# AleoNet/snarkVM

Measured on AMD Instinct MI355X. Metric: BLS12-377 G1 MSM scalar-point pairs/sec (+ Fr NTT elements/sec in ntt_*), higher is better.
Workload: dtype u32 limbs (29-bit radix) modular integer arithmetic, Fq 377-bit / Fr 253-bit; 1 GPU; G1 Pippenger MSM 2^24 (BASELINE.json configs[1]), bases (i+1)G registered in HBM, uniform scalars in HBM; independent instance per GPU; scalars=uniform, lg_ntt=24, window_bits=auto, base_tables=12, table_bits=22, pipelined_batch=True

## Files before the change

include/snarkvm_hip.h:

```cpp
#ifndef SNARKVM_HIP_H
#define SNARKVM_HIP_H

#include <stddef.h>
#include <stdint.h>

#ifdef __cplusplus
extern "C" {
#endif

typedef struct {
    int32_t code;
    char *message;
} RustError;

enum NTTInputOutputOrder { NN = 0, NR = 1, RN = 2, RR = 3 };
enum NTTDirection { Forward = 0, Inverse = 1 };
enum NTTType { Standard = 0, Coset = 1 };


RustError snarkvm_ntt(void *inout, uint32_t lg_domain_size, enum NTTInputOutputOrder ntt_order,
                      enum NTTDirection ntt_direction, enum NTTType ntt_type);

RustError snarkvm_polymul(void *out, size_t pcount, const void *polynomials, const void *plens, size_t ecount,
                          const void *evaluations, const void *elens, uint32_t lg_domain_size);

RustError snarkvm_msm(void *out, const void *points_with_infinity, size_t npoints, const void *scalars,
                      size_t ffi_affine_sz);
RustError snarkvm_hip_set_base_cache(int tables);
RustError snarkvm_hip_set_base_cache_verified(int tables);
void snarkvm_hip_base_cache_stats(uint64_t *out, int reset);


int snarkvm_hip_device_count(void);
int snarkvm_hip_batch_lanes(size_t npoints);
RustError snarkvm_hip_set_devices(const int32_t *ids, size_t n);
RustError snarkvm_hip_set_device(int device);
int snarkvm_hip_num_devices(void);

RustError snarkvm_hip_malloc(void **d_ptr, size_t bytes, int device);
RustError snarkvm_hip_free(void *d_ptr);
RustError snarkvm_hip_memcpy_h2d(void *d_dst, const void *src, size_t bytes);
RustError snarkvm_hip_memcpy_d2h(void *dst, const void *d_src, size_t bytes);
RustError snarkvm_hip_memcpy_d2d(void *d_dst, const void *d_src, size_t bytes);
RustError snarkvm_hip_memset(void *d_dst, int value, size_t bytes);

RustError snarkvm_hip_ntt_device(void *d_inout, uint32_t lg_domain_size, int ntt_order, int ntt_direction,
                                 int ntt_type);
RustError snarkvm_hip_ntt_device_batch(void *const *d_inouts, size_t count, uint32_t lg_domain_size, int ntt_order,
                                       const int *ntt_directions, const int *ntt_types);

RustError snarkvm_hip_polymul_device(void *d_out, size_t pcount, const void *const *d_polys, const size_t *plens, size_t ecount,
                                     const void *const *d_evals, const size_t *elens, uint32_t lg_domain_size);

RustError snarkvm_hip_scope_begin(const void *d_any);
RustError snarkvm_hip_scope_end(void);
enum { SNARKVM_HIP_SCOPE_ASYNC_MSM = 1, SNARKVM_HIP_SCOPE_STABLE_INPUTS = 2, SNARKVM_HIP_SCOPE_MSM_IN_STREAM = 4 };
RustError snarkvm_hip_scope_begin_ex(const void *d_any, uint32_t flags);
RustError snarkvm_hip_scope_collect(const void *out);
RustError snarkvm_hip_scope_set_flags(uint32_t flags);
void *snarkvm_hip_scope_stream(void);

typedef struct snarkvm_hip_bases snarkvm_hip_bases_t;
RustError snarkvm_hip_register_bases(snarkvm_hip_bases_t **handle, const void *points, size_t npoints,
                                     size_t ffi_affine_sz, int on_device);
RustError snarkvm_hip_register_bases_tables(snarkvm_hip_bases_t **handle, const void *points, size_t npoints,
                                            size_t ffi_affine_sz, int on_device, int tables);
RustError snarkvm_hip_register_bases_windowed(snarkvm_hip_bases_t **handle, const void *points, size_t npoints,
                                              size_t ffi_affine_sz, int on_device, int tables, int window_bits);
void snarkvm_hip_free_bases(snarkvm_hip_bases_t *handle);

RustError snarkvm_hip_register_bases_serialized(snarkvm_hip_bases_t **handle, const void *bytes, size_t npoints,
                                                int compressed, int validate, int tables);
RustError snarkvm_hip_g1_deserialize(void *out_affine, const void *bytes, size_t n, int compressed, int validate);
RustError snarkvm_hip_g1_serialize(void *out_bytes, const void *affine, size_t n, size_t ffi_affine_sz, int compressed);

RustError snarkvm_hip_g2_deserialize(void *out_affine, const void *bytes, size_t n, int validate);
RustError snarkvm_hip_g2_serialize(void *out_bytes, const void *affine, size_t n, size_t ffi_affine_sz);
RustError snarkvm_hip_g2_deserialize_compressed(void *out_affine, const void *bytes, size_t n, int validate);
RustError snarkvm_hip_g2_serialize_compressed(void *out_bytes, const void *affine, size_t n, size_t ffi_affine_sz);

RustError snarkvm_hip_msm_registered(void *out, const snarkvm_hip_bases_t *handle, size_t offset, size_t npoints,
                                     const void *scalars, int scalars_on_device, int window_bits);

RustError snarkvm_hip_msm_registered_ex(void *out, const snarkvm_hip_bases_t *handle, size_t off0, size_t n0,
                                        size_t off1, size_t n1, const void *scalars, int scalars_on_device,
                                        int scalars_montgomery, int window_bits);

RustError snarkvm_hip_msm_registered_batch(void *outs, const snarkvm_hip_bases_t *handle, size_t count,
                                           const size_t *offsets, const size_t *npoints, const void *const *scalars,
                                           int scalars_on_device, int scalars_montgomery, int window_bits);

RustError snarkvm_hip_msm_registered_batch_ex(void *outs, const snarkvm_hip_bases_t *handle, size_t count, const size_t *off0,
                                              const size_t *n0, const size_t *off1, const size_t *n1,
                                              const void *const *scalars, int scalars_on_device, int scalars_montgomery,
                                              int window_bits);

RustError snarkvm_hip_g1_sum(void *out, const void *in_projective, size_t n);

RustError snarkvm_hip_g1_to_affine(void *out_affine, const void *in_projective, size_t n);

RustError snarkvm_hip_msm_g2(void *out, const void *points_with_infinity, size_t npoints, const void *scalars,
                             size_t ffi_affine_sz);

typedef struct snarkvm_hip_bases_g2 snarkvm_hip_bases_g2_t;
RustError snarkvm_hip_register_bases_g2(snarkvm_hip_bases_g2_t **handle, const void *points, size_t npoints,
                                        size_t ffi_affine_sz, int tables, int window_bits);
void snarkvm_hip_free_bases_g2(snarkvm_hip_bases_g2_t *handle);
RustError snarkvm_hip_msm_g2_registered(void *out, const snarkvm_hip_bases_g2_t *handle, size_t offset, size_t npoints,
                                        const void *scalars, int scalars_on_device, int window_bits);
RustError snarkvm_hip_msm_g2_registered_batch(void *outs, const snarkvm_hip_bases_g2_t *handle, size_t count,
                                              const size_t *offsets, const size_t *npoints, const void *const *scalars,
                                              int scalars_on_device, int window_bits);

RustError snarkvm_hip_g1_fixed_base_msm(void *out_projective, const void *g_affine, const void *scalars, size_t n);
RustError snarkvm_hip_g1_group_ntt(void *inout_projective, uint32_t lg_domain_size, int inverse);

RustError snarkvm_hip_fr_mul_device(void *d_out, const void *d_a, const void *d_b, size_t n);
RustError snarkvm_hip_fr_convert_device(void *d_out, const void *d_in, size_t n, int to_bigint);

RustError snarkvm_hip_fr_vec_op(int op, void *out, const void *a, const void *b, const void *c, const void *scalar,
                                size_t n, int on_device);
RustError snarkvm_hip_fr_divide_by_linear(void *quotient, void *remainder, const void *poly, size_t n,
                                          const void *point, int on_device);
RustError snarkvm_hip_fr_batch_inversion_and_mul(void *inout, size_t n, const void *coeff, int on_device);
RustError snarkvm_hip_fr_distribute_powers(void *inout, size_t n, const void *g, const void *c, int on_device);
RustError snarkvm_hip_fr_lagrange_coefficients(void *out, uint32_t lg_domain_size, const void *tau, int on_device);
RustError snarkvm_hip_fr_divide_by_vanishing(void *quotient, void *remainder, const void *poly, size_t len,
                                             size_t domain_size, int on_device);
RustError snarkvm_hip_fr_mul_by_vanishing(void *out, const void *poly, size_t len, size_t domain_size, int on_device);

RustError snarkvm_hip_fr_lincomb(void *out, size_t n_out, size_t count, const void *const *polys, const size_t *lens, const void *coeffs,
                                 int on_device);

RustError snarkvm_hip_fr_vec_op_strided(int op, void *out, const void *a, const void *b, const void *c, const void *scalar,
                                        size_t n, size_t count, size_t stride);
RustError snarkvm_hip_fr_divide_by_linear_strided(void *quotients, void *remainders, const void *polys, size_t n,
                                                  const void *point, size_t count, size_t stride);
RustError snarkvm_hip_fr_divide_by_vanishing_strided(void *quotients, void *remainders, const void *polys, size_t len,
                                                     size_t domain_size, size_t count, size_t stride);

RustError snarkvm_hip_g1_generate_bases_device(void *d_out, uint64_t start, size_t npoints);

void snarkvm_hip_set_profiling(int enabled);
int snarkvm_hip_get_phase_count(void);
const char *snarkvm_hip_get_phase_name(int i);
double snarkvm_hip_get_phase_ms(int i);

void snarkvm_hip_coalescer_stats(uint64_t *out, int reset);

void snarkvm_hip_alloc_stats(uint64_t *out, int reset);

RustError snarkvm_hip_synchronize(void);


int snarkvm_hip_selftest_field(int field, int op, const void *a, const void *b, void *out, size_t n);
int snarkvm_hip_selftest_g1_msm_naive(const void *points_with_infinity, size_t npoints, size_t ffi_affine_sz,
                                      const void *scalars, void *out);
int snarkvm_hip_selftest_msm_plan(size_t n, int window_bits, int tables, int table_bits, uint32_t *out);
int snarkvm_hip_selftest_g1_finish(const void *planes_projective, const int32_t *pos, size_t n, void *out);
int snarkvm_hip_selftest_fq_lazy(uint64_t seed, int iters);
int snarkvm_hip_selftest_g1_lazy_tail(uint64_t seed, int iters);
int snarkvm_hip_selftest_fq2_pair(const void *points, size_t npoints, uint64_t seed, int iters);
int snarkvm_hip_selftest_g2_hex(const void *points, size_t npoints, uint64_t seed, int iters);
RustError snarkvm_hip_devtest_g2_tail_repeat(const void *points, size_t npoints, int m, int hb, int threads, int plane_threads,
                                             int hex, int quads, int iters, uint32_t *report);
int snarkvm_hip_selftest_ntt_plan(uint32_t lg, int32_t *out);
int snarkvm_hip_selftest_ntt_twiddle(int kind, uint32_t lg, int pass, int inverse, const uint64_t *x, size_t n, void *out);
int snarkvm_hip_selftest_ntt_index(uint32_t lg, const int32_t *plan, int npass);
int snarkvm_hip_selftest_ntt_host(void *inout, uint32_t lg, const int32_t *plan, int npass, int dir, int type);
int snarkvm_hip_selftest_fr_lincomb(void *out, size_t n_out, size_t count, const void *const *polys, const size_t *lens, const void *coeffs);
RustError snarkvm_hip_devtest_field(int field, int op, const void *a, const void *b, void *out, size_t n);

#ifdef __cplusplus
}
#endif
#endif
```

rust/snarkvm-algorithms-hip/src/sys.rs:

```rust
#![allow(non_camel_case_types, non_snake_case, clippy::too_many_arguments, clippy::missing_safety_doc)]
use super::{Error, NTTDirection, NTTInputOutputOrder, NTTType};
use core::ffi::{c_char, c_void};

#[repr(C)]
pub struct snarkvm_hip_bases_t {
    _private: [u8; 0],
}
#[repr(C)]
pub struct snarkvm_hip_bases_g2_t {
    _private: [u8; 0],
}

pub const SNARKVM_HIP_SCOPE_ASYNC_MSM: u32 = 1;
pub const SNARKVM_HIP_SCOPE_STABLE_INPUTS: u32 = 2;
pub const SNARKVM_HIP_SCOPE_MSM_IN_STREAM: u32 = 4;

extern "C" {
    pub fn snarkvm_ntt(inout: *mut c_void, lg_domain_size: u32, ntt_order: NTTInputOutputOrder, ntt_direction: NTTDirection, ntt_type: NTTType) -> Error;
    pub fn snarkvm_polymul(out: *mut c_void, pcount: usize, polynomials: *const c_void, plens: *const c_void, ecount: usize, evaluations: *const c_void, elens: *const c_void, lg_domain_size: u32) -> Error;
    pub fn snarkvm_msm(out: *mut c_void, points_with_infinity: *const c_void, npoints: usize, scalars: *const c_void, ffi_affine_sz: usize) -> Error;
    pub fn snarkvm_hip_set_base_cache(tables: i32) -> Error;
    pub fn snarkvm_hip_set_base_cache_verified(tables: i32) -> Error;
    pub fn snarkvm_hip_base_cache_stats(out: *mut u64, reset: i32);
    pub fn snarkvm_hip_device_count() -> i32;
    pub fn snarkvm_hip_batch_lanes(npoints: usize) -> i32;
    pub fn snarkvm_hip_set_devices(ids: *const i32, n: usize) -> Error;
    pub fn snarkvm_hip_set_device(device: i32) -> Error;
    pub fn snarkvm_hip_num_devices() -> i32;
    pub fn snarkvm_hip_malloc(d_ptr: *mut *mut c_void, bytes: usize, device: i32) -> Error;
    pub fn snarkvm_hip_free(d_ptr: *mut c_void) -> Error;
    pub fn snarkvm_hip_memcpy_h2d(d_dst: *mut c_void, src: *const c_void, bytes: usize) -> Error;
    pub fn snarkvm_hip_memcpy_d2h(dst: *mut c_void, d_src: *const c_void, bytes: usize) -> Error;
    pub fn snarkvm_hip_memcpy_d2d(d_dst: *mut c_void, d_src: *const c_void, bytes: usize) -> Error;
    pub fn snarkvm_hip_memset(d_dst: *mut c_void, value: i32, bytes: usize) -> Error;
    pub fn snarkvm_hip_ntt_device(d_inout: *mut c_void, lg_domain_size: u32, ntt_order: i32, ntt_direction: i32, ntt_type: i32) -> Error;
    pub fn snarkvm_hip_ntt_device_batch(d_inouts: *const *mut c_void, count: usize, lg_domain_size: u32, ntt_order: i32, ntt_directions: *const i32, ntt_types: *const i32) -> Error;
    pub fn snarkvm_hip_polymul_device(d_out: *mut c_void, pcount: usize, d_polys: *const *const c_void, plens: *const usize, ecount: usize, d_evals: *const *const c_void, elens: *const usize, lg_domain_size: u32) -> Error;
    pub fn snarkvm_hip_scope_begin(d_any: *const c_void) -> Error;
    pub fn snarkvm_hip_scope_end() -> Error;
    pub fn snarkvm_hip_scope_begin_ex(d_any: *const c_void, flags: u32) -> Error;
    pub fn snarkvm_hip_scope_collect(out: *const c_void) -> Error;
    pub fn snarkvm_hip_scope_set_flags(flags: u32) -> Error;
    pub fn snarkvm_hip_scope_stream() -> *mut c_void;
    pub fn snarkvm_hip_register_bases(handle: *mut *mut snarkvm_hip_bases_t, points: *const c_void, npoints: usize, ffi_affine_sz: usize, on_device: i32) -> Error;
    pub fn snarkvm_hip_register_bases_tables(handle: *mut *mut snarkvm_hip_bases_t, points: *const c_void, npoints: usize, ffi_affine_sz: usize, on_device: i32, tables: i32) -> Error;
    pub fn snarkvm_hip_register_bases_windowed(handle: *mut *mut snarkvm_hip_bases_t, points: *const c_void, npoints: usize, ffi_affine_sz: usize, on_device: i32, tables: i32, window_bits: i32) -> Error;
    pub fn snarkvm_hip_free_bases(handle: *mut snarkvm_hip_bases_t);
    pub fn snarkvm_hip_register_bases_serialized(handle: *mut *mut snarkvm_hip_bases_t, bytes: *const c_void, npoints: usize, compressed: i32, validate: i32, tables: i32) -> Error;
    pub fn snarkvm_hip_g1_deserialize(out_affine: *mut c_void, bytes: *const c_void, n: usize, compressed: i32, validate: i32) -> Error;
    pub fn snarkvm_hip_g1_serialize(out_bytes: *mut c_void, affine: *const c_void, n: usize, ffi_affine_sz: usize, compressed: i32) -> Error;
    pub fn snarkvm_hip_g2_deserialize(out_affine: *mut c_void, bytes: *const c_void, n: usize, validate: i32) -> Error;
    pub fn snarkvm_hip_g2_serialize(out_bytes: *mut c_void, affine: *const c_void, n: usize, ffi_affine_sz: usize) -> Error;
    pub fn snarkvm_hip_g2_deserialize_compressed(out_affine: *mut c_void, bytes: *const c_void, n: usize, validate: i32) -> Error;
    pub fn snarkvm_hip_g2_serialize_compressed(out_bytes: *mut c_void, affine: *const c_void, n: usize, ffi_affine_sz: usize) -> Error;
    pub fn snarkvm_hip_msm_registered(out: *mut c_void, handle: *const snarkvm_hip_bases_t, offset: usize, npoints: usize, scalars: *const c_void, scalars_on_device: i32, window_bits: i32) -> Error;
    pub fn snarkvm_hip_msm_registered_ex(out: *mut c_void, handle: *const snarkvm_hip_bases_t, off0: usize, n0: usize, off1: usize, n1: usize, scalars: *const c_void, scalars_on_device: i32, scalars_montgomery: i32, window_bits: i32) -> Error;
    pub fn snarkvm_hip_msm_registered_batch(outs: *mut c_void, handle: *const snarkvm_hip_bases_t, count: usize, offsets: *const usize, npoints: *const usize, scalars: *const *const c_void, scalars_on_device: i32, scalars_montgomery: i32, window_bits: i32) -> Error;
    pub fn snarkvm_hip_msm_registered_batch_ex(outs: *mut c_void, handle: *const snarkvm_hip_bases_t, count: usize, off0: *const usize, n0: *const usize, off1: *const usize, n1: *const usize, scalars: *const *const c_void, scalars_on_device: i32, scalars_montgomery: i32, window_bits: i32) -> Error;
    pub fn snarkvm_hip_g1_sum(out: *mut c_void, in_projective: *const c_void, n: usize) -> Error;
    pub fn snarkvm_hip_g1_to_affine(out_affine: *mut c_void, in_projective: *const c_void, n: usize) -> Error;
    pub fn snarkvm_hip_msm_g2(out: *mut c_void, points_with_infinity: *const c_void, npoints: usize, scalars: *const c_void, ffi_affine_sz: usize) -> Error;
    pub fn snarkvm_hip_register_bases_g2(handle: *mut *mut snarkvm_hip_bases_g2_t, points: *const c_void, npoints: usize, ffi_affine_sz: usize, tables: i32, window_bits: i32) -> Error;
    pub fn snarkvm_hip_free_bases_g2(handle: *mut snarkvm_hip_bases_g2_t);
    pub fn snarkvm_hip_msm_g2_registered(out: *mut c_void, handle: *const snarkvm_hip_bases_g2_t, offset: usize, npoints: usize, scalars: *const c_void, scalars_on_device: i32, window_bits: i32) -> Error;
    pub fn snarkvm_hip_msm_g2_registered_batch(outs: *mut c_void, handle: *const snarkvm_hip_bases_g2_t, count: usize, offsets: *const usize, npoints: *const usize, scalars: *const *const c_void, scalars_on_device: i32, window_bits: i32) -> Error;
    pub fn snarkvm_hip_g1_fixed_base_msm(out_projective: *mut c_void, g_affine: *const c_void, scalars: *const c_void, n: usize) -> Error;
    pub fn snarkvm_hip_g1_group_ntt(inout_projective: *mut c_void, lg_domain_size: u32, inverse: i32) -> Error;
    pub fn snarkvm_hip_fr_mul_device(d_out: *mut c_void, d_a: *const c_void, d_b: *const c_void, n: usize) -> Error;
    pub fn snarkvm_hip_fr_convert_device(d_out: *mut c_void, d_in: *const c_void, n: usize, to_bigint: i32) -> Error;
    pub fn snarkvm_hip_fr_vec_op(op: i32, out: *mut c_void, a: *const c_void, b: *const c_void, c: *const c_void, scalar: *const c_void, n: usize, on_device: i32) -> Error;
    pub fn snarkvm_hip_fr_divide_by_linear(quotient: *mut c_void, remainder: *mut c_void, poly: *const c_void, n: usize, point: *const c_void, on_device: i32) -> Error;
    pub fn snarkvm_hip_fr_batch_inversion_and_mul(inout: *mut c_void, n: usize, coeff: *const c_void, on_device: i32) -> Error;
    pub fn snarkvm_hip_fr_distribute_powers(inout: *mut c_void, n: usize, g: *const c_void, c: *const c_void, on_device: i32) -> Error;
    pub fn snarkvm_hip_fr_lagrange_coefficients(out: *mut c_void, lg_domain_size: u32, tau: *const c_void, on_device: i32) -> Error;
    pub fn snarkvm_hip_fr_divide_by_vanishing(quotient: *mut c_void, remainder: *mut c_void, poly: *const c_void, len: usize, domain_size: usize, on_device: i32) -> Error;
    pub fn snarkvm_hip_fr_mul_by_vanishing(out: *mut c_void, poly: *const c_void, len: usize, domain_size: usize, on_device: i32) -> Error;
    pub fn snarkvm_hip_fr_lincomb(out: *mut c_void, n_out: usize, count: usize, polys: *const *const c_void, lens: *const usize, coeffs: *const c_void, on_device: i32) -> Error;
    pub fn snarkvm_hip_fr_vec_op_strided(op: i32, out: *mut c_void, a: *const c_void, b: *const c_void, c: *const c_void, scalar: *const c_void, n: usize, count: usize, stride: usize) -> Error;
    pub fn snarkvm_hip_fr_divide_by_linear_strided(quotients: *mut c_void, remainders: *mut c_void, polys: *const c_void, n: usize, point: *const c_void, count: usize, stride: usize) -> Error;
    pub fn snarkvm_hip_fr_divide_by_vanishing_strided(quotients: *mut c_void, remainders: *mut c_void, polys: *const c_void, len: usize, domain_size: usize, count: usize, stride: usize) -> Error;
    pub fn snarkvm_hip_g1_generate_bases_device(d_out: *mut c_void, start: u64, npoints: usize) -> Error;
    pub fn snarkvm_hip_set_profiling(enabled: i32);
    pub fn snarkvm_hip_get_phase_count() -> i32;
    pub fn snarkvm_hip_get_phase_name(i: i32) -> *const c_char;
    pub fn snarkvm_hip_get_phase_ms(i: i32) -> f64;
    pub fn snarkvm_hip_coalescer_stats(out: *mut u64, reset: i32);
    pub fn snarkvm_hip_alloc_stats(out: *mut u64, reset: i32);
    pub fn snarkvm_hip_synchronize() -> Error;
    pub fn snarkvm_hip_selftest_field(field: i32, op: i32, a: *const c_void, b: *const c_void, out: *mut c_void, n: usize) -> i32;
    pub fn snarkvm_hip_selftest_g1_msm_naive(points_with_infinity: *const c_void, npoints: usize, ffi_affine_sz: usize, scalars: *const c_void, out: *mut c_void) -> i32;
    pub fn snarkvm_hip_selftest_msm_plan(n: usize, window_bits: i32, tables: i32, table_bits: i32, out: *mut u32) -> i32;
    pub fn snarkvm_hip_selftest_g1_finish(planes_projective: *const c_void, pos: *const i32, n: usize, out: *mut c_void) -> i32;
    pub fn snarkvm_hip_selftest_fq_lazy(seed: u64, iters: i32) -> i32;
    pub fn snarkvm_hip_selftest_g1_lazy_tail(seed: u64, iters: i32) -> i32;
    pub fn snarkvm_hip_selftest_fq2_pair(points: *const c_void, npoints: usize, seed: u64, iters: i32) -> i32;
    pub fn snarkvm_hip_selftest_g2_hex(points: *const c_void, npoints: usize, seed: u64, iters: i32) -> i32;
    pub fn snarkvm_hip_devtest_g2_tail_repeat(points: *const c_void, npoints: usize, m: i32, hb: i32, threads: i32, plane_threads: i32, hex: i32, quads: i32, iters: i32, report: *mut u32) -> Error;
    pub fn snarkvm_hip_selftest_ntt_plan(lg: u32, out: *mut i32) -> i32;
    pub fn snarkvm_hip_selftest_ntt_twiddle(kind: i32, lg: u32, pass: i32, inverse: i32, x: *const u64, n: usize, out: *mut c_void) -> i32;
    pub fn snarkvm_hip_selftest_ntt_index(lg: u32, plan: *const i32, npass: i32) -> i32;
    pub fn snarkvm_hip_selftest_ntt_host(inout: *mut c_void, lg: u32, plan: *const i32, npass: i32, dir: i32, type_: i32) -> i32;
    pub fn snarkvm_hip_selftest_fr_lincomb(out: *mut c_void, n_out: usize, count: usize, polys: *const *const c_void, lens: *const usize, coeffs: *const c_void) -> i32;
    pub fn snarkvm_hip_devtest_field(field: i32, op: i32, a: *const c_void, b: *const c_void, out: *mut c_void, n: usize) -> Error;
}
```

snarkvm_amd/_lib.py:

```python
import ctypes
import os

_HERE = os.path.dirname(os.path.abspath(__file__))
LIB_PATH = os.environ.get("SNARKVM_HIP_LIB") or os.path.join(_HERE, "lib", "libsnarkvm_hip.so")

SYMBOLS = [
    "snarkvm_ntt", "snarkvm_polymul", "snarkvm_msm", "snarkvm_hip_set_base_cache", "snarkvm_hip_set_base_cache_verified", "snarkvm_hip_base_cache_stats",
    "snarkvm_hip_device_count", "snarkvm_hip_batch_lanes", "snarkvm_hip_set_device", "snarkvm_hip_set_devices", "snarkvm_hip_num_devices",
    "snarkvm_hip_malloc", "snarkvm_hip_free", "snarkvm_hip_memcpy_h2d", "snarkvm_hip_memcpy_d2h", "snarkvm_hip_memcpy_d2d", "snarkvm_hip_memset", "snarkvm_hip_ntt_device", "snarkvm_hip_ntt_device_batch", "snarkvm_hip_polymul_device",
    "snarkvm_hip_scope_begin", "snarkvm_hip_scope_end", "snarkvm_hip_scope_begin_ex", "snarkvm_hip_scope_collect", "snarkvm_hip_scope_set_flags", "snarkvm_hip_scope_stream", "snarkvm_hip_alloc_stats",
    "snarkvm_hip_register_bases", "snarkvm_hip_register_bases_tables", "snarkvm_hip_register_bases_windowed", "snarkvm_hip_free_bases", "snarkvm_hip_msm_registered", "snarkvm_hip_msm_g2",
    "snarkvm_hip_msm_registered_ex", "snarkvm_hip_msm_registered_batch", "snarkvm_hip_msm_registered_batch_ex", "snarkvm_hip_g1_to_affine",
    "snarkvm_hip_fr_mul_device", "snarkvm_hip_fr_convert_device", "snarkvm_hip_g1_generate_bases_device",
    "snarkvm_hip_fr_vec_op", "snarkvm_hip_fr_divide_by_linear", "snarkvm_hip_fr_batch_inversion_and_mul",
    "snarkvm_hip_fr_distribute_powers", "snarkvm_hip_fr_lagrange_coefficients", "snarkvm_hip_fr_divide_by_vanishing",
    "snarkvm_hip_fr_mul_by_vanishing", "snarkvm_hip_fr_lincomb",
    "snarkvm_hip_fr_vec_op_strided", "snarkvm_hip_fr_divide_by_linear_strided", "snarkvm_hip_fr_divide_by_vanishing_strided",
    "snarkvm_hip_register_bases_serialized", "snarkvm_hip_g1_deserialize", "snarkvm_hip_g1_serialize", "snarkvm_hip_g1_sum", "snarkvm_hip_g2_deserialize", "snarkvm_hip_g2_serialize", "snarkvm_hip_g2_deserialize_compressed", "snarkvm_hip_g2_serialize_compressed",
    "snarkvm_hip_register_bases_g2", "snarkvm_hip_free_bases_g2", "snarkvm_hip_msm_g2_registered", "snarkvm_hip_msm_g2_registered_batch",
    "snarkvm_hip_g1_fixed_base_msm", "snarkvm_hip_g1_group_ntt",
    "snarkvm_hip_set_profiling", "snarkvm_hip_get_phase_count", "snarkvm_hip_get_phase_name",
    "snarkvm_hip_get_phase_ms", "snarkvm_hip_synchronize", "snarkvm_hip_coalescer_stats",
    "snarkvm_hip_selftest_field", "snarkvm_hip_selftest_g1_msm_naive", "snarkvm_hip_selftest_msm_plan", "snarkvm_hip_selftest_g1_finish", "snarkvm_hip_selftest_fq_lazy", "snarkvm_hip_selftest_g1_lazy_tail", "snarkvm_hip_selftest_ntt_plan", "snarkvm_hip_selftest_ntt_twiddle", "snarkvm_hip_selftest_ntt_index", "snarkvm_hip_selftest_ntt_host", "snarkvm_hip_selftest_fq2_pair", "snarkvm_hip_selftest_g2_hex", "snarkvm_hip_selftest_fr_lincomb", "snarkvm_hip_devtest_field", "snarkvm_hip_devtest_g2_tail_repeat",
]


class RustError(ctypes.Structure):
    _fields_ = [("code", ctypes.c_int32), ("message", ctypes.c_void_p)]


class HipError(RuntimeError):
    def __init__(self, code, message):
        super().__init__(f"snarkvm_hip error {code}: {message}")
        self.code = code
        self.message = message


_lib = None
_libc = None


def lib():
    global _lib, _libc
    if _lib is None:
        if not os.path.exists(LIB_PATH):
            raise ImportError(
                f"{LIB_PATH} is missing - build it with `python -m snarkvm_amd.build` (hipcc, gfx950). "
                "snarkvm_amd has no CPU fallback.")
        if not os.environ.get("SNARKVM_HIP_NO_TORCH"):
            try:
                import torch
            except ImportError:
                pass
        L = ctypes.CDLL(LIB_PATH)
        err_fns = ["snarkvm_ntt", "snarkvm_polymul", "snarkvm_msm", "snarkvm_hip_set_base_cache", "snarkvm_hip_set_base_cache_verified", "snarkvm_hip_set_device", "snarkvm_hip_set_devices",
                   "snarkvm_hip_malloc", "snarkvm_hip_free", "snarkvm_hip_memcpy_h2d", "snarkvm_hip_memcpy_d2h", "snarkvm_hip_memcpy_d2d", "snarkvm_hip_memset", "snarkvm_hip_ntt_device", "snarkvm_hip_ntt_device_batch", "snarkvm_hip_polymul_device",
                   "snarkvm_hip_scope_begin", "snarkvm_hip_scope_end", "snarkvm_hip_scope_begin_ex", "snarkvm_hip_scope_collect", "snarkvm_hip_scope_set_flags",
                   "snarkvm_hip_register_bases", "snarkvm_hip_register_bases_tables", "snarkvm_hip_register_bases_windowed", "snarkvm_hip_msm_registered", "snarkvm_hip_msm_g2", "snarkvm_hip_msm_registered_ex", "snarkvm_hip_msm_registered_batch", "snarkvm_hip_msm_registered_batch_ex", "snarkvm_hip_g1_to_affine", "snarkvm_hip_fr_mul_device",
                   "snarkvm_hip_fr_convert_device", "snarkvm_hip_g1_generate_bases_device", "snarkvm_hip_synchronize",
                   "snarkvm_hip_fr_vec_op", "snarkvm_hip_fr_divide_by_linear", "snarkvm_hip_fr_batch_inversion_and_mul", "snarkvm_hip_fr_distribute_powers", "snarkvm_hip_fr_lagrange_coefficients", "snarkvm_hip_fr_divide_by_vanishing", "snarkvm_hip_fr_mul_by_vanishing", "snarkvm_hip_fr_lincomb",
                   "snarkvm_hip_fr_vec_op_strided", "snarkvm_hip_fr_divide_by_linear_strided", "snarkvm_hip_fr_divide_by_vanishing_strided",
                   "snarkvm_hip_register_bases_serialized", "snarkvm_hip_g1_deserialize", "snarkvm_hip_g1_serialize", "snarkvm_hip_g1_sum", "snarkvm_hip_g2_deserialize", "snarkvm_hip_g2_serialize", "snarkvm_hip_g2_deserialize_compressed", "snarkvm_hip_g2_serialize_compressed",
                   "snarkvm_hip_register_bases_g2", "snarkvm_hip_msm_g2_registered", "snarkvm_hip_msm_g2_registered_batch",
                   "snarkvm_hip_g1_fixed_base_msm", "snarkvm_hip_g1_group_ntt",
                   "snarkvm_hip_devtest_field", "snarkvm_hip_devtest_g2_tail_repeat"]
        for name in err_fns:
            getattr(L, name).restype = RustError
        L.snarkvm_hip_device_count.restype = ctypes.c_int
        L.snarkvm_hip_batch_lanes.restype = ctypes.c_int
        L.snarkvm_hip_num_devices.restype = ctypes.c_int
        L.snarkvm_hip_selftest_g1_finish.restype = ctypes.c_int
        L.snarkvm_hip_selftest_fq_lazy.restype = ctypes.c_int
        L.snarkvm_hip_selftest_g1_lazy_tail.restype = ctypes.c_int
        for name in ("snarkvm_hip_selftest_ntt_plan", "snarkvm_hip_selftest_ntt_twiddle", "snarkvm_hip_selftest_ntt_index", "snarkvm_hip_selftest_ntt_host"):
            getattr(L, name).restype = ctypes.c_int
        L.snarkvm_hip_selftest_fq2_pair.restype = ctypes.c_int
        L.snarkvm_hip_selftest_g2_hex.restype = ctypes.c_int
        L.snarkvm_hip_selftest_fr_lincomb.restype = ctypes.c_int
        L.snarkvm_hip_get_phase_count.restype = ctypes.c_int
        L.snarkvm_hip_get_phase_name.restype = ctypes.c_char_p
        L.snarkvm_hip_get_phase_ms.restype = ctypes.c_double
        L.snarkvm_hip_selftest_field.restype = ctypes.c_int
        L.snarkvm_hip_selftest_g1_msm_naive.restype = ctypes.c_int
        L.snarkvm_hip_selftest_msm_plan.restype = ctypes.c_int
        L.snarkvm_hip_free_bases.restype = None
        L.snarkvm_hip_free_bases_g2.restype = None
        L.snarkvm_hip_set_profiling.restype = None
        L.snarkvm_hip_coalescer_stats.restype = None
        L.snarkvm_hip_base_cache_stats.restype = None
        L.snarkvm_hip_alloc_stats.restype = None
        L.snarkvm_hip_scope_stream.restype = ctypes.c_void_p
        L.snarkvm_hip_scope_begin_ex.argtypes = [ctypes.c_void_p, ctypes.c_uint32]
        L.snarkvm_hip_scope_set_flags.argtypes = [ctypes.c_uint32]
        L.snarkvm_hip_alloc_stats.argtypes = [ctypes.c_void_p, ctypes.c_int]
        L.snarkvm_hip_coalescer_stats.argtypes = [ctypes.c_void_p, ctypes.c_int]
        L.snarkvm_hip_base_cache_stats.argtypes = [ctypes.c_void_p, ctypes.c_int]
        L.snarkvm_hip_malloc.argtypes = [ctypes.POINTER(ctypes.c_void_p), ctypes.c_size_t, ctypes.c_int]
        L.snarkvm_hip_free.argtypes = [ctypes.c_void_p]
        L.snarkvm_hip_memcpy_h2d.argtypes = [ctypes.c_void_p, ctypes.c_void_p, ctypes.c_size_t]
        L.snarkvm_hip_memcpy_d2h.argtypes = [ctypes.c_void_p, ctypes.c_void_p, ctypes.c_size_t]
        L.snarkvm_hip_memcpy_d2d.argtypes = [ctypes.c_void_p, ctypes.c_void_p, ctypes.c_size_t]
        L.snarkvm_hip_memset.argtypes = [ctypes.c_void_p, ctypes.c_int, ctypes.c_size_t]
        L.snarkvm_hip_polymul_device.argtypes = [ctypes.c_void_p, ctypes.c_size_t, ctypes.POINTER(ctypes.c_void_p), ctypes.POINTER(ctypes.c_size_t),
                                                 ctypes.c_size_t, ctypes.POINTER(ctypes.c_void_p), ctypes.POINTER(ctypes.c_size_t), ctypes.c_uint32]
        L.snarkvm_hip_fr_lincomb.argtypes = [ctypes.c_void_p, ctypes.c_size_t, ctypes.c_size_t, ctypes.POINTER(ctypes.c_void_p), ctypes.POINTER(ctypes.c_size_t),
                                             ctypes.c_void_p, ctypes.c_int]
        L.snarkvm_hip_selftest_fr_lincomb.argtypes = L.snarkvm_hip_fr_lincomb.argtypes[:-1]
        _libc = ctypes.CDLL(None)
        _libc.free.argtypes = [ctypes.c_void_p]
        _lib = L
    return _lib


def check(err):
    if err.code != 0:
        msg = ctypes.string_at(err.message).decode(errors="replace") if err.message else ""
        if err.message:
            _libc.free(err.message)
        raise HipError(err.code, msg)


def device_count():
    return lib().snarkvm_hip_device_count()
```

snarkvm_amd/csrc/api.hip:

```cpp
#define SV_TU_G1
#include "runtime.hip.h"
#include "ffl.hip.h"

runtime_t g_rt;
thread_local thread_scope_t g_tl_scope;
thread_scope_t::~thread_scope_t() {
    if (!lane) return;
    pending.clear();
    (void)hipStreamSynchronize(lane->stream);
    for (int i = 0; i < naux; i++) {
        (void)hipStreamSynchronize(aux[i]->stream);
        aux[i]->dev->give(aux[i], true);
    }
    lane->in_scope = false;
    lane->deferred.clear();
    lane->deferred_bytes = 0;
    if (!lane->tw_leases.empty()) ntt_tw_release(lane->dev, lane->tw_leases);
    lane->dev->give(lane, true);
    lane = nullptr;
}
std::atomic<uint64_t> g_co_stats[4];
static std::atomic<uint64_t> g_alloc_stats[5];
void sv_alloc_note(int slot, size_t bytes, double ms) {
    g_alloc_stats[slot].fetch_add(1, std::memory_order_relaxed);
// ... 153 lines not shown
    c.sync_or_defer();
    API_END
}

static constexpr uint32_t SCOPE_FLAGS_ALL = SNARKVM_HIP_SCOPE_ASYNC_MSM | SNARKVM_HIP_SCOPE_STABLE_INPUTS | SNARKVM_HIP_SCOPE_MSM_IN_STREAM;
RustError snarkvm_hip_scope_begin_ex(const void* d_any, uint32_t flags) {
    API_TRY
    thread_scope_t& sc = tl_scope();
    if (sc.lane) throw hip_failure{hipErrorInvalidValue, "scope_begin: the calling thread already has an open scope", __LINE__};
    if (flags & ~SCOPE_FLAGS_ALL) throw hip_failure{hipErrorInvalidValue, "scope_begin: unknown flag", __LINE__};
    g_rt.configure();
    const int nd = (int)g_rt.devs.size();
    int dev = device_for(d_any, d_any ? 1 : 0);
    if (dev < 0) dev = (int)(g_rt.rr.fetch_add(1) % (uint32_t)nd);
    device_t* d = g_rt.devs[dev].get();
    int prev = -1;
    if (hipGetDevice(&prev) != hipSuccess) prev = 0;
    lane_t* l = d->take_for_scope(true);
    try {
        HIP_TRY(hipSetDevice(d->physical));
        d->init();
        tu_kernel_attributes(d->logical);
    } catch (...) {
        d->give(l, true);
        (void)hipSetDevice(prev);
        throw;
    }
    l->begin_call();
    l->in_scope = true;
    l->pin_used = 0;
    l->scope_events_used = 0;
    sc = thread_scope_t();
    sc.lane = l;
    sc.prev_device = prev;
    sc.flags = flags;
    API_CATCH
}
RustError snarkvm_hip_scope_begin(const void* d_any) { return snarkvm_hip_scope_begin_ex(d_any, 0); }
void* snarkvm_hip_scope_stream(void) {
    lane_t* l = tl_scope().lane;
    return l ? (void*)l->stream : nullptr;
}
RustError snarkvm_hip_scope_set_flags(uint32_t flags) {
    API_TRY
    thread_scope_t& sc = tl_scope();
    if (!sc.lane) throw hip_failure{hipErrorInvalidValue, "scope_set_flags: the calling thread has no open scope", __LINE__};
    if (flags & ~SCOPE_FLAGS_ALL) throw hip_failure{hipErrorInvalidValue, "scope_set_flags: unknown flag", __LINE__};
    sc.flags = flags;
    API_CATCH
}
RustError snarkvm_hip_scope_collect(const void* out) {
    API_TRY
    scope_collect(out);
    API_CATCH
}
RustError snarkvm_hip_scope_end(void) {
    thread_scope_t& sc = tl_scope();
    lane_t* l = sc.lane;
    if (!l) return ok();
    RustError r = ok();
    try {
        scope_flush();
    } catch (const hip_failure& f) {
        r = from_failure(f);
    } catch (const std::exception& e) {
        r = fail(1, std::string("snarkvm_hip: scope_end: ") + e.what());
    } catch (...) {
        r = fail(1, "snarkvm_hip: scope_end failed");
    }
    l->in_scope = false;
    l->deferred.clear();
    l->deferred_bytes = 0;
    for (int i = 0; i < sc.naux; i++) {
        (void)hipStreamSynchronize(sc.aux[i]->stream);
        sc.aux[i]->dev->give(sc.aux[i], true);
    }
    const int prev = sc.prev_device;
    sc = thread_scope_t();
    l->dev->give(l, true);
    if (prev >= 0) (void)hipSetDevice(prev);
    return r;
}

static void precompute_tables(lane_t& c, snarkvm_hip_bases* h, g1_aff_mem_t* d) { precompute_tables_run<fq_t>(c, d, h->n, h->tables, h->table_bits); }
static void register_bases_impl(snarkvm_hip_bases_t** handle, const void* points, size_t npoints, size_t ffi_affine_sz, int on_device, int tables,
                                int table_bits) {
    if (!handle) throw hip_failure{hipErrorInvalidValue, "register_bases: null handle", __LINE__};
    if (npoints && !points) throw hip_failure{hipErrorInvalidValue, "register_bases: null points", __LINE__};
    if (ffi_affine_sz < 104 || (ffi_affine_sz & 7)) throw hip_failure{hipErrorInvalidValue, "register_bases: bad stride", __LINE__};
    check_tables(tables, table_bits, "register_bases");
    scope_flush();
    const int nd = g_rt.ndev();
    std::unique_ptr<snarkvm_hip_bases> h(new snarkvm_hip_bases());
    h->n = npoints;
    h->tables = tables;
    h->table_bits = table_bits ? table_bits : 256 / tables;
    h->d.assign(nd, nullptr);
    const size_t bytes = (size_t)tables * npoints * sizeof(g1_aff_mem_t);
    try {
        if (npoints) {
            const int owner = on_device ? device_for(points, 1) : -1;
            auto build = [&](int dev) {
                lane_guard lg(dev);
                lane_t& c = lg.c();
                HIP_TRY(hipMalloc((void**)&h->d[dev], bytes));
                const uint8_t* src = (const uint8_t*)points;
                if (!on_device) {
                    c.bases_tmp.ensure(npoints * ffi_affine_sz);
                    HIP_TRY(hipMemcpyAsync(c.bases_tmp.p, points, npoints * ffi_affine_sz, hipMemcpyHostToDevice, c.stream));
                    src = c.bases_tmp.as<uint8_t>();
                }
                convert_bases<fq_t>(c, src, ffi_affine_sz, npoints, h->d[dev]);
                precompute_tables(c, h.get(), h->d[dev]);
                bases_to_lazy_form(c, h->d[dev], (size_t)tables * npoints);
                HIP_TRY(hipStreamSynchronize(c.stream));
            };
            std::vector<int> all;
            for (int d = 0; d < nd; d++) all.push_back(d);
            if (!on_device) {
                for_each_device(all, build);
            } else {
                build(owner);
                for (int d = 0; d < nd; d++) {
                    if (d == owner) continue;
                    lane_guard lg(d);
                    HIP_TRY(hipMalloc((void**)&h->d[d], bytes));
                    HIP_TRY(hipMemcpyPeerAsync(h->d[d], g_rt.devs[d]->physical, h->d[owner], g_rt.devs[owner]->physical, bytes, lg.c().stream));
                    HIP_TRY(hipStreamSynchronize(lg.c().stream));
                }
            }
        }
    } catch (...) {
        h->free_all();
        throw;
    }
    *handle = h.release();
}
RustError snarkvm_hip_register_bases(snarkvm_hip_bases_t** handle, const void* points, size_t npoints, size_t ffi_affine_sz, int on_device) {
    API_TRY
    register_bases_impl(handle, points, npoints, ffi_affine_sz, on_device, 1, 0);
    API_CATCH
}
RustError snarkvm_hip_register_bases_tables(snarkvm_hip_bases_t** handle, const void* points, size_t npoints, size_t ffi_affine_sz, int on_device,
                                            int tables) {
    API_TRY
    register_bases_impl(handle, points, npoints, ffi_affine_sz, on_device, tables, 0);
    API_CATCH
}
RustError snarkvm_hip_register_bases_windowed(snarkvm_hip_bases_t** handle, const void* points, size_t npoints, size_t ffi_affine_sz, int on_device,
                                              int tables, int window_bits) {
    API_TRY
    if (window_bits <= 0) throw hip_failure{hipErrorInvalidValue, "register_bases_windowed: window_bits must be positive", __LINE__};
    register_bases_impl(handle, points, npoints, ffi_affine_sz, on_device, tables, window_bits);
    API_CATCH
}
void snarkvm_hip_free_bases(snarkvm_hip_bases_t* h) {
    if (!h) return;
    h->free_all();
    delete h;
}
}
snarkvm_hip_bases* sv_new_bases_handle(size_t npoints, int tables, int table_bits) {
    snarkvm_hip_bases* h = new snarkvm_hip_bases();
    h->n = npoints;
    h->tables = tables;
    h->table_bits = table_bits;
    h->d.assign(g_rt.ndev(), nullptr);
    return h;
}
void sv_precompute_tables(lane_t& c, snarkvm_hip_bases* h, g1_aff_mem_t* d) { precompute_tables(c, h, d); }
extern "C" {

static void check_window_bits(int window_bits, const char* who) {
    if (window_bits && (window_bits < 2 || window_bits > MSM_C_MAX)) throw std::runtime_error(std::string(who) + ": window_bits must be 0 or 2..23");
}
static void msm_registered_host_scalars(void* out, const snarkvm_hip_bases* h, size_t off0, size_t n0, size_t off1, size_t n1, const void* scalars,
                                        int scalars_montgomery, int window_bits) {
    const size_t n = n0 + n1;
    scope_flush();
    const int nd = g_rt.ndev();
    static const int trace = getenv("SNARKVM_HIP_TRACE") ? atoi(getenv("SNARKVM_HIP_TRACE")) : 0;
    const double t_begin = host_now_ms();
    size_t parts = n / MSM_SPLIT_MIN;
    if (parts > (size_t)nd) parts = (size_t)nd;
    if (parts < 1) parts = 1;
    const size_t chunk = msm_scalar_chunk_pairs();
    if (n >= 2 * chunk && (n + chunk - 1) / chunk > parts) parts = (n + chunk - 1) / chunk;
    std::vector<size_t> bound;
    const int geo = tuning().scalar_geo;
    if (nd == 1 && geo > 1 && tuning().taper != 0 && n >= ((size_t)1 << 22)) {
        parts = n >= ((size_t)1 << 23) ? 3 : 2;
        size_t wsum = 0, w = 1;
        for (size_t i = 0; i < parts; i++, w *= (size_t)geo) wsum += w;
        size_t acc_w = 0;
        w = 1;
        bound.push_back(0);
        for (size_t i = 0; i < parts; i++, w *= (size_t)geo) {
            acc_w += w;
            bound.push_back(i + 1 == parts ? n : (size_t)((unsigned __int128)n * acc_w / wsum));
        }
    } else {
        for (size_t i = 0; i <= parts; i++) bound.push_back(n * i / parts);
    }
    const int ndu = (int)(parts < (size_t)nd ? parts : (size_t)nd);
    std::unique_ptr<msm_accum_t<fq_t>> acc(new msm_accum_t<fq_t>());
    std::mutex acc_mu;
    std::vector<int> devs;
    if (ndu == 1) {
        devs.push_back(-1);
    } else {
        for (int d = 0; d < ndu; d++) devs.push_back(d);
    }
    const size_t slot = msm_plane_bytes<fq_t>();
    for_each_device(devs, [&](int dev) {
        std::vector<size_t> mine;
        for (size_t i = (dev < 0 ? 0 : (size_t)dev); i < parts; i += (size_t)ndu) mine.push_back(i);
        lane_guard lg;
        lg.acquire(dev, mine.size() > 2 ? 3 : (int)mine.size());
        const size_t L = lg.lanes.size();
        size_t max_cnt = 0;
        for (size_t j = 0; j < mine.size(); j++) {
            const size_t cnt = bound[mine[j] + 1] - bound[mine[j]];
            max_cnt = cnt > max_cnt ? cnt : max_cnt;
        }
        const bool use_sink = tuning().taper != 0 && mine.size() >= 2;
        std::vector<msm_pending_t> pend(use_sink ? 1 : mine.size());
        int chunk_c = window_bits;
        msm_bucket_sink_t sink;
        std::vector<hipEvent_t> merged;
        for (size_t l = 0; l < L; l++) {
            lane_t& c = *lg.lanes[l];
            c.begin_call();
            c.scalars_tmp.ensure(max_cnt * 32 + 32);
            c.pin.ensure(slot * (use_sink ? 1 : (mine.size() + L - 1) / L));
        }
        if (use_sink) {
            lane_t& c0 = *lg.lanes[0];
            const msm_plan_t pl = msm_make_plan(max_cnt, window_bits, h->tables, h->table_bits);
// ... 615 lines not shown
        }
    }
    const g1_jac_t j = total.to_jacobian();
    uint32_t* o = (uint32_t*)out;
    j.x.to_mem_mont().pack(o);
    j.y.to_mem_mont().pack(o + 12);
    j.z.to_mem_mont().pack(o + 24);
    return 0;
}
int snarkvm_hip_selftest_fq_lazy(uint64_t seed, int iters) {
    uint32_t xw[12], yw[12];
    memcpy(xw, G1_GEN_X, 48);
    memcpy(yw, G1_GEN_Y, 48);
    const g1_aff_t g{fq_t::unpack(xw).from_mem_mont(), fq_t::unpack(yw).from_mem_mont()};
    std::vector<g1_aff_t> pool;
    g1_xyzz_t run = g1_xyzz_t::inf();
    for (int k = 0; k < 64; k++) {
        run.add_affine(g);
        const fq_t izzz = run.zzz.inverse();
        const fq_t izz = izzz.sqr() * run.zz.sqr();
        pool.push_back({run.x * izz, run.y * izzz});
    }
    const fq_t c406 = fq_t::from_table(FqLConv::C406), c348 = fq_t::from_table(FqLConv::C348);
    auto next = [&]() {
        seed += 0x9E3779B97F4A7C15ull;
        uint64_t z = seed;
        z = (z ^ (z >> 30)) * 0xBF58476D1CE4E5B9ull;
        z = (z ^ (z >> 27)) * 0x94D049BB133111EBull;
        return z ^ (z >> 31);
    };
    g1_xyzz_t exact = g1_xyzz_t::inf();
    xyzz_lazy_t lazy = xyzz_lazy_t::infinity();
    int prev = -1;
    bool prev_neg = false;
    for (int it = 0; it < iters; it++) {
        const uint64_t r = next();
        int k = (int)(r % 64);
        bool neg = ((r >> 8) & 1) != 0;
        const int mode = (int)((r >> 16) % 16);
        if (mode == 0 && prev >= 0) k = prev, neg = prev_neg;
        if (mode == 1 && prev >= 0) k = prev, neg = !prev_neg;
        if (mode == 2) {
            exact = g1_xyzz_t::inf();
            lazy = xyzz_lazy_t::infinity();
        }
        prev = k;
        prev_neg = neg;
        const g1_aff_t p = pool[k];
        exact.add_affine(p, neg);
        const fql_t px = fql_t::from_limbs(p.x * c406), py = fql_t::from_limbs(p.y * c406);
        if (!lazy.madd(px, py, neg)) {
            g1_xyzz_t e = lazy.to_exact();
            fq_t ex, ey;
            for (int i = 0; i < 13; i++) ex.v[i] = (uint32_t)px.v[i], ey.v[i] = (uint32_t)py.v[i];
            e.add_affine({ex * c348, ey * c348}, neg);
            lazy = xyzz_lazy_t::from_exact(e);
        }
        const g1_xyzz_t got = lazy.to_exact();
        if (got.is_inf() != exact.is_inf()) return it + 1;
        if (!exact.is_inf() && (got.x != exact.x || got.y != exact.y || got.zz != exact.zz || got.zzz != exact.zzz)) return it + 1;
    }
    for (int t = 0; t < 200; t++) {
        fq_t a, b;
        for (int i = 0; i < 13; i++) a.v[i] = (uint32_t)(next() & LIMB_MASK), b.v[i] = (uint32_t)(next() & LIMB_MASK);
        a.v[12] &= 0x00ffffffu;
        b.v[12] &= 0x00ffffffu;
        if (t & 1) for (int i = 0; i < 12; i++) a.v[i] = LIMB_MASK;
        if (t & 2) for (int i = 0; i < 12; i++) b.v[i] = (i & 1) ? LIMB_MASK : 0;
        const fql_t la = fql_t::from_exact(a), lb = fql_t::from_exact(b);
        if (fql_t::mul(la, lb).to_exact() != a * b) return -(4 * t + 1);
        if (fql_t::sqr(la - lb).to_exact() != (a - b).sqr()) return -(4 * t + 2);
        if (fql_t::diff_of_products(la - lb, lb - la, fql_t::from_exact(a * b).normalized(), la).to_exact() != fq_t::diff_of_products(a - b, b - a, a * b, a))
            return -(4 * t + 3);
        if (((la + lb) - (lb + lb)).normalized().to_exact() != (a - b)) return -(4 * t + 4);
        alignas(16) uint32_t raw[12];
        const fql_t wide = (la - lb - lb - lb).normalized();
        wide.store_raw(raw);
        const fql_t back = fql_t::load_raw(raw);
        for (int i = 0; i < 13; i++)
            if (back.v[i] != wide.v[i]) return -(100000 + t);
    }
    return 0;
}
int snarkvm_hip_selftest_g1_lazy_tail(uint64_t seed, int iters) {
    uint32_t xw[12], yw[12];
    memcpy(xw, G1_GEN_X, 48);
    memcpy(yw, G1_GEN_Y, 48);
    const g1_aff_t g{fq_t::unpack(xw).from_mem_mont(), fq_t::unpack(yw).from_mem_mont()};
    std::vector<g1_xyzz_t> pool;
    g1_xyzz_t run = g1_xyzz_t::inf();
    for (int k = 0; k < 48; k++) {
        run.add_affine(g);
        pool.push_back(run);
    }
    auto next = [&]() {
        seed += 0x9E3779B97F4A7C15ull;
        uint64_t z = seed;
        z = (z ^ (z >> 30)) * 0xBF58476D1CE4E5B9ull;
        z = (z ^ (z >> 27)) * 0x94D049BB133111EBull;
        return z ^ (z >> 31);
    };
    auto to_lazy = [](const g1_xyzz_t& p) {
        xyzz_t<fqz_t> r = xyzz_t<fqz_t>::inf();
        if (!p.is_inf()) r = {{fql_t::from_exact(p.x)}, {fql_t::from_exact(p.y)}, {fql_t::from_exact(p.zz)}, {fql_t::from_exact(p.zzz)}};
        return r;
    };
    g1_xyzz_t exact = g1_xyzz_t::inf();
    xyzz_t<fqz_t> lazy = xyzz_t<fqz_t>::inf();
    g1_xyzz_t prev = g1_xyzz_t::inf();
    for (int it = 0; it < iters; it++) {
        const uint64_t r = next();
        g1_xyzz_t p = pool[r % 48];
        fq_t l = fq_t::zero();
        for (int i = 0; i < 12; i++) l.v[i] = (uint32_t)(next() & LIMB_MASK);
        l.v[0] |= 1;
        const fq_t l2 = l.sqr(), l3 = l2 * l;
        p = {p.x * l2, p.y * l3, p.zz * l2, p.zzz * l3};
        if ((r >> 8) & 1) p.y = p.y.neg();
        const int mode = (int)((r >> 16) % 16);
        if (mode == 0) p = prev;
        if (mode == 1) p = {prev.x, prev.y.neg(), prev.zz, prev.zzz};
        if (mode == 2) {
            exact = g1_xyzz_t::inf();
            lazy = xyzz_t<fqz_t>::inf();
        }
        if (mode == 3) p = exact;
        if (mode == 4) {
            exact = exact.dbl();
            lazy = lazy.dbl();
        } else {
            prev = p;
            exact.add(p);
            lazy.add(to_lazy(p));
        }
        if (lazy.is_inf() != exact.is_inf()) return it + 1;
        if (!exact.is_inf() && (lazy.x.to_exact() != exact.x || lazy.y.to_exact() != exact.y || lazy.zz.to_exact() != exact.zz || lazy.zzz.to_exact() != exact.zzz))
            return it + 1;
        xyzz_mem_t<fqz_t> m;
        store_xyzz<fqz_t>(&m, lazy);
        lazy = load_xyzz<fqz_t>(&m);
    }
    fqz_t zq;
    for (int i = 0; i < 13; i++) zq.a.v[i] = FqL::MOD[i];
    if (!zq.is_zero() || !zq.neg().is_zero() || !(zq + zq).is_zero() || (zq + fqz_t::one()).is_zero()) return -1;
    return 0;
}
int snarkvm_hip_selftest_g1_finish(const void* planes_jacobian, const int32_t* pos, size_t n, void* out) {
    try {
        std::unique_ptr<msm_accum_t<fq_t>> acc(new msm_accum_t<fq_t>());
        const uint32_t* src = (const uint32_t*)planes_jacobian;
        for (size_t i = 0; i < n; i++) {
            const g1_jac_t j = {fq_t::from_raw_words(src + 36 * i), fq_t::from_raw_words(src + 36 * i + 12), fq_t::from_raw_words(src + 36 * i + 24)};
            acc->add(pos[i], g1_xyzz_t::from_jacobian(j));
        }
        acc->finish(out);
        return 0;
    } catch (...) {
        return 1;
    }
}

}
```

snarkvm_amd/csrc/api_serde.hip:

```cpp
#include "runtime.hip.h"

snarkvm_hip_bases* sv_new_bases_handle(size_t npoints, int tables, int table_bits);
void sv_precompute_tables(lane_t& c, snarkvm_hip_bases* h, g1_aff_mem_t* d);

static uint32_t g1_deserialize_run(lane_t& c, const void* bytes, size_t n, int compressed, int validate, g1_aff_mem_t* d_native, uint8_t* d_rust) {
    const size_t psz = compressed ? 48 : 96;
    c.bases_tmp.ensure(n * psz);
    c.serde_status.ensure(4);
    HIP_TRY(hipMemcpyAsync(c.bases_tmp.p, bytes, n * psz, hipMemcpyHostToDevice, c.stream));
    HIP_TRY(hipMemsetAsync(c.serde_status.p, 0, 4, c.stream));
    hipLaunchKernelGGL(g1_deserialize_kernel, dim3((unsigned)((n + 63) / 64)), dim3(64), 0, c.stream, c.bases_tmp.as<uint8_t>(), n, compressed, validate,
                       d_native, d_rust, c.serde_status.as<uint32_t>());
    HIP_TRY(hipGetLastError());
    uint32_t st = 0;
    HIP_TRY(hipMemcpyAsync(&st, c.serde_status.p, 4, hipMemcpyDeviceToHost, c.stream));
    HIP_TRY(hipStreamSynchronize(c.stream));
    return st;
}

extern "C" {

RustError snarkvm_hip_register_bases_serialized(snarkvm_hip_bases_t** handle, const void* bytes, size_t npoints, int compressed, int validate,
                                                int tables) {
    API_TRY
    if (!handle || (npoints && !bytes)) throw hip_failure{hipErrorInvalidValue, "register_bases_serialized: null argument", __LINE__};
    check_tables(tables, 0, "register_bases_serialized");
    std::unique_ptr<snarkvm_hip_bases> h(sv_new_bases_handle(npoints, tables, 256 / tables));
    if (npoints) {
        try {
            std::vector<int> all;
            for (int d = 0; d < g_rt.ndev(); d++) all.push_back(d);
            for_each_device(all, [&](int dev) {
                lane_guard lg(dev);
                lane_t& c = lg.c();
                HIP_TRY(hipMalloc((void**)&h->d[dev], (size_t)tables * npoints * sizeof(g1_aff_mem_t)));
                serde_throw_on_status(g1_deserialize_run(c, bytes, npoints, compressed, validate, h->d[dev], nullptr), "register_bases_serialized");
                sv_precompute_tables(c, h.get(), h->d[dev]);
                bases_to_lazy_form(c, h->d[dev], (size_t)tables * npoints);
                HIP_TRY(hipStreamSynchronize(c.stream));
            });
        } catch (...) {
            h->free_all();
            throw;
        }
    }
    *handle = h.release();
    API_CATCH
}
RustError snarkvm_hip_g1_deserialize(void* out_affine, const void* bytes, size_t n, int compressed, int validate) {
    API_BEGIN
    if (n) {
        if (!out_affine || !bytes) throw hip_failure{hipErrorInvalidValue, "g1_deserialize: null argument", __LINE__};
        c.poly[0].ensure(n * 104);
        const uint32_t st = g1_deserialize_run(c, bytes, n, compressed, validate, nullptr, c.poly[0].as<uint8_t>());
        serde_throw_on_status(st, "g1_deserialize");
        HIP_TRY(hipMemcpyAsync(out_affine, c.poly[0].p, n * 104, hipMemcpyDeviceToHost, c.stream));
        HIP_TRY(hipStreamSynchronize(c.stream));
    }
    API_END
}
RustError snarkvm_hip_g1_serialize(void* out_bytes, const void* affine, size_t n, size_t ffi_affine_sz, int compressed) {
    API_BEGIN
    if (n) {
        if (!out_bytes || !affine) throw hip_failure{hipErrorInvalidValue, "g1_serialize: null argument", __LINE__};
        if (ffi_affine_sz < 104 || (ffi_affine_sz & 7)) throw hip_failure{hipErrorInvalidValue, "g1_serialize: bad stride", __LINE__};
        const size_t psz = compressed ? 48 : 96;
        c.bases_tmp.ensure(n * ffi_affine_sz);
        c.poly[0].ensure(n * psz);
        HIP_TRY(hipMemcpyAsync(c.bases_tmp.p, affine, n * ffi_affine_sz, hipMemcpyHostToDevice, c.stream));
        hipLaunchKernelGGL(g1_serialize_kernel, dim3((unsigned)((n + 63) / 64)), dim3(64), 0, c.stream, c.bases_tmp.as<uint8_t>(), ffi_affine_sz, n,
                           compressed, c.poly[0].as<uint8_t>());
        HIP_TRY(hipGetLastError());
        HIP_TRY(hipMemcpyAsync(out_bytes, c.poly[0].p, n * psz, hipMemcpyDeviceToHost, c.stream));
        HIP_TRY(hipStreamSynchronize(c.stream));
    }
    API_END
}

}
```

snarkvm_amd/csrc/msm_sort.hip.h:

```cpp
#pragma once
#include "ffl.hip.h"
#include "ffl2.hip.h"
#include "ffl2p.hip.h"
#include "msm.hip.h"

namespace sv {

static constexpr int SORT_TILE = 8192;
static constexpr int SORT_THREADS = 256;

struct msm_inst_t {
    const uint4* scalars;
    uint32_t n;
    uint32_t n0;
    uint32_t off0, off1;
    uint32_t pstart;
    uint32_t ptiles;
};
struct msm_radix_params_t {
    size_t n;
    int c, W, J;
    int HB, LB;
    uint32_t nb;
    uint32_t tiles_per_row;
    uint32_t TPW;
    const msm_inst_t* inst = nullptr;
    uint32_t ninst = 0;
    uint32_t vstride = 0, vn0 = 0, vr0 = 0, vr1 = 0;
    uint32_t xcd = 0;
};
__device__ __forceinline__ uint32_t xcd_tile(uint32_t b, uint32_t T) {
    const uint32_t q = T >> 3, r = T & 7u, x = b & 7u;
    return (x < r ? x * (q + 1) : r * (q + 1) + (x - r) * q) + (b >> 3);
}
struct l1_tile_t {
    uint32_t w, tw, TPW, j;
    size_t cbase;
    size_t row;
    size_t lo, hi;
    uint32_t inst_idx;
};
__device__ __forceinline__ l1_tile_t l1_decode_tile(const msm_radix_params_t& p, uint32_t g) {
    l1_tile_t t;
    const uint32_t B1 = 1u << p.HB;
    if (!p.inst) {
        t.w = g / p.TPW;
        t.tw = g - t.w * p.TPW;
        t.TPW = p.TPW;
        t.j = t.tw / p.tiles_per_row;
        const uint32_t tt = t.tw - t.j * p.tiles_per_row;
        t.cbase = (size_t)t.w * B1 * p.TPW;
        t.row = (size_t)(t.j * p.W + t.w) * p.n;
        t.lo = (size_t)tt * SORT_TILE;
        t.hi = (t.lo + SORT_TILE < p.n) ? t.lo + SORT_TILE : p.n;
        t.inst_idx = 0;
        return t;
    }
    const uint32_t J = (uint32_t)p.J;
    uint32_t lo = 0, hi = p.ninst;
    while (hi - lo > 1) {
        const uint32_t mid = (lo + hi) >> 1;
        if (J * (p.inst[mid].pstart / SORT_TILE) <= g) lo = mid; else hi = mid;
    }
    const msm_inst_t in = p.inst[lo];
    const uint32_t tw0 = J * (in.pstart / SORT_TILE);
    t.w = lo;
    t.inst_idx = lo;
    t.tw = g - tw0;
    t.TPW = J * in.ptiles;
    t.j = t.tw / in.ptiles;
    const uint32_t tt = t.tw - t.j * in.ptiles;
    t.cbase = (size_t)B1 * tw0;
    t.row = (size_t)t.j * p.n;
    t.lo = (size_t)in.pstart + (size_t)tt * SORT_TILE;
    t.hi = t.lo + SORT_TILE;
    return t;
}

__device__ __forceinline__ bool digit_bucket(uint32_t u, int half, uint32_t& b, uint32_t& neg) {
    const int dv = (int)u - half;
    if (dv == 0) return false;
    neg = dv < 0 ? 0x80000000u : 0u;
    b = (uint32_t)((dv < 0 ? -dv : dv) - 1);
    return true;
}

// ... 631 lines not shown
            raw = raw_next;
            if (pos + 1 < hi) {
                e_next = sorted[pos + 1];
                raw_next = *slot_of(e_next);
            }
        } else {
            raw = *slot_of(e);
            if (pos + 1 < hi) e_next = sorted[pos + 1];
        }
        acc.add_affine(load_aff<F>(&raw), (e >> 31) != 0);
    }
    store_xyzz<F>(&partial[start_k + part_off], acc);
}

static __global__ void __launch_bounds__(256) g1_partials_to_exact_kernel(const g1_lazy_partial_t* __restrict__ raw, g1_xyzz_mem_t* __restrict__ partial,
                                                                   const uint32_t* __restrict__ start, uint32_t nbt) {
    const uint32_t i = blockIdx.x * blockDim.x + threadIdx.x;
    if (i >= start[nbt]) return;
    g1_store_xyzz(&partial[i], xyzz_lazy_t::exact_from_raw(&raw[i]));
}
static __device__ __noinline__ void lazy_exceptional_add(xyzz_lazy_t* acc, const fql_t* px, const fql_t* py, bool neg) {
    g1_xyzz_t ex = acc->to_exact();
    const fq_t c348 = fq_t::from_table(FqLConv::C348);
    fq_t bx, by;
#pragma unroll
    for (int i = 0; i < 13; i++) bx.v[i] = (uint32_t)px->v[i], by.v[i] = (uint32_t)py->v[i];
    ex.add_affine({bx * c348, by * c348}, neg);
    *acc = xyzz_lazy_t::from_exact(ex);
}
template <bool PREFETCH>
__global__ void __launch_bounds__(256, 1) msm_accumulate_lazy_kernel(const g1_aff_mem_t* __restrict__ bases, const uint32_t* __restrict__ sorted,
                                                              const uint32_t* __restrict__ boff, const uint32_t* __restrict__ start,
                                                              g1_lazy_partial_t* __restrict__ partial, uint32_t nbt, uint32_t S, uint32_t debug_idx_mask) {
    const uint32_t t = blockIdx.x * blockDim.x + threadIdx.x;
    const uint32_t total = boff[nbt];
    const uint64_t lo64 = (uint64_t)t * S;
    if (lo64 >= total) return;
    const uint32_t lo = (uint32_t)lo64;
    const uint32_t hi = (total - lo < S) ? total : lo + S;
    uint32_t k = find_bucket(boff, nbt, lo);
    uint32_t kend = boff[k + 1];
    uint32_t kend2 = boff[k + 2 <= nbt ? k + 2 : nbt];
    uint32_t start_k = start[k];
    uint32_t part_off = t - boff[k] / S;
    xyzz_lazy_t acc = xyzz_lazy_t::infinity();
    auto slot_of = [&](uint32_t e) -> const g1_lazy_slot_t* { return (const g1_lazy_slot_t*)&bases[(e & 0x7fffffffu) & debug_idx_mask]; };
    uint32_t e_cur = sorted[lo];
    uint32_t e_n1 = lo + 1 < hi ? sorted[lo + 1] : 0u;
    g1_lazy_slot_t raw_next = *slot_of(e_cur);
    for (uint32_t pos = lo;; pos++) {
        const bool end = pos >= hi;
        if (end || pos >= kend) {
            acc.store_raw(&partial[start_k + part_off]);
            if (end) break;
            part_off = 0;
            acc.inf = true;
            k++;
            kend = kend2;
            while (pos >= kend) {
                k++;
                kend = boff[k + 1];
            }
            kend2 = boff[k + 2 <= nbt ? k + 2 : nbt];
            start_k = start[k];
        }
        const uint32_t e = e_cur;
        const g1_lazy_slot_t raw = raw_next;
        if (pos + 1 < hi) raw_next = *slot_of(e_n1);
        e_cur = e_n1;
        if (pos + 2 < hi) e_n1 = sorted[pos + 2];
        if (raw.w[26]) continue;
        const bool neg = (e >> 31) != 0;
        fql_t px, py;
        raw.coords(px, py);
        if (!acc.madd(px, py, neg)) {
            xyzz_lazy_t tmp = acc;
            const fql_t tx = px, ty = py;
            lazy_exceptional_add(&tmp, &tx, &ty, neg);
            acc = tmp;
        }
    }
}

static __global__ void __launch_bounds__(256) g2_pair_partials_to_exact_kernel(const g2_pair_partial_t* __restrict__ raw, xyzz_mem_t<fq2_t>* __restrict__ partial,
                                                                        const uint32_t* __restrict__ start, uint32_t nbt) {
    const uint32_t g = blockIdx.x * blockDim.x + threadIdx.x;
    const uint32_t i = g >> 3, k = g & 7;
    if (i >= start[nbt]) return;
    const uint4* q = (const uint4*)&raw[i].w[16 * k];
    uint32_t t[16];
#pragma unroll
    for (int j = 0; j < 4; j++) {
        const uint4 u = q[j];
        t[4 * j] = u.x, t[4 * j + 1] = u.y, t[4 * j + 2] = u.z, t[4 * j + 3] = u.w;
    }
    fql_t c;
#pragma unroll
    for (int j = 0; j < 13; j++) c.v[j] = (int32_t)t[j];
    c.to_exact().store(&((fq_mem_t*)&partial[i])[k]);
}
template <bool PREFETCH>
__global__ void __launch_bounds__(256, 2) msm_accumulate_pair2_kernel(const aff_mem_t<fq2_t>* __restrict__ bases, const uint32_t* __restrict__ sorted,
                                                               const uint32_t* __restrict__ boff, const uint32_t* __restrict__ start,
                                                               g2_pair_partial_t* __restrict__ partial, uint32_t nbt, uint32_t S, uint32_t debug_idx_mask) {
    const uint32_t gt = blockIdx.x * blockDim.x + threadIdx.x;
    const uint32_t t = gt >> 1;
    const int comp = (int)(gt & 1u);
    const uint32_t total = boff[nbt];
    const uint64_t lo64 = (uint64_t)t * S;
    if (lo64 >= total) return;
    const uint32_t lo = (uint32_t)lo64;
    const uint32_t hi = (total - lo < S) ? total : lo + S;
    uint32_t k = find_bucket(boff, nbt, lo);
    uint32_t kend = boff[k + 1];
    uint32_t start_k = start[k];
    uint32_t part_off = t - boff[k] / S;
    fq2p::xyzz_pair_t<fq2p::xp_dev> acc;
    acc.inf = true;
    auto slot_of = [&](uint32_t e) -> const g2_lazy_slot_t* { return (const g2_lazy_slot_t*)&bases[(e & 0x7fffffffu) & debug_idx_mask]; };
    for (uint32_t pos = lo;; pos++) {
        const bool end = pos >= hi;
        if (end || pos >= kend) {
            uint4* q = (uint4*)&partial[start_k + part_off].w[16 * comp];
            if (acc.inf) {
#pragma unroll
                for (int c4 = 0; c4 < 4; c4++)
#pragma unroll
                    for (int j = 0; j < 4; j++) q[8 * c4 + j] = make_uint4(0, 0, 0, 0);
            } else {
                const fql_t* cs[4] = {&acc.x[0], &acc.y[0], &acc.zz[0], &acc.zzz[0]};
#pragma unroll
                for (int c4 = 0; c4 < 4; c4++) {
                    const int32_t* v = cs[c4]->v;
                    q[8 * c4 + 0] = make_uint4((uint32_t)v[0], (uint32_t)v[1], (uint32_t)v[2], (uint32_t)v[3]);
                    q[8 * c4 + 1] = make_uint4((uint32_t)v[4], (uint32_t)v[5], (uint32_t)v[6], (uint32_t)v[7]);
                    q[8 * c4 + 2] = make_uint4((uint32_t)v[8], (uint32_t)v[9], (uint32_t)v[10], (uint32_t)v[11]);
                    q[8 * c4 + 3] = make_uint4((uint32_t)v[12], 0u, 0u, 0u);
                }
            }
            if (end) break;
            part_off = 0;
            acc.inf = true;
            do {
                k++;
                kend = boff[k + 1];
            } while (pos >= kend);
            start_k = start[k];
        }
        const uint32_t e = sorted[pos];
        const g2_lazy_slot_t* sp = slot_of(e);
        if (sp->w[g2_lazy_slot_t::INF_WORD]) continue;
        fql_t px[1], py[1];
        sp->component(comp, px[0], py[0]);
        acc.madd(px, py, (e >> 31) != 0);
    }
}

}
```

snarkvm_amd/csrc/runtime.hip.h:

```cpp
#pragma once
#include <hip/hip_runtime.h>
#include <stdint.h>
#include <stdio.h>
#include <stdlib.h>
#include <string.h>
#include <time.h>

#include <atomic>
#include <chrono>
#include <condition_variable>
#include <deque>
#include <functional>
#include <exception>
#include <memory>
#include <mutex>
#include <stdexcept>
#include <string>
#include <thread>
#include <type_traits>
#include <utility>
#include <vector>

#include "../../include/snarkvm_hip.h"
#include "ec.hip.h"
// ... 272 lines not shown
                return &lane[l];
            }
        }
        return nullptr;
    }
    void give(lane_t* l, bool from_scope = false) {
        {
            std::lock_guard<std::mutex> lk(mu);
            busy &= ~(1u << l->index);
            if (from_scope) scope_held--;
        }
        cv.notify_all();
    }
};

struct runtime_t {
    std::mutex cfg_mu;
    std::vector<int> want;
    std::vector<std::unique_ptr<device_t>> devs;
    bool configured = false;
    std::atomic<uint32_t> rr{0};
    std::atomic<bool> profiling{false};
    std::mutex prof_mu;
    std::vector<std::pair<std::string, double>> last_phases;

    void configure() {
        std::lock_guard<std::mutex> lk(cfg_mu);
        if (configured) return;
        int ndev = 0;
        hipError_t e = hipGetDeviceCount(&ndev);
        if (e != hipSuccess || ndev == 0) throw hip_failure{e == hipSuccess ? hipErrorNoDevice : e, "hipGetDeviceCount (no MI355X visible)", __LINE__};
        std::vector<int> ids = want;
        if (ids.empty()) {
            if (const char* env = getenv("SNARKVM_HIP_DEVICES")) {
                for (const char* p = env; *p;) {
                    char* end = nullptr;
                    long v = strtol(p, &end, 10);
                    if (end == p) break;
                    ids.push_back((int)v);
                    p = (*end == ',') ? end + 1 : end;
                }
            }
        }
        if (ids.empty())
            for (int d = 0; d < ndev; d++) ids.push_back(d);
        for (int id : ids)
            if (id < 0 || id >= ndev) throw hip_failure{hipErrorInvalidDevice, "device index out of range (snarkvm_hip_set_devices / SNARKVM_HIP_DEVICES)", __LINE__};
        for (size_t i = 0; i < ids.size(); i++) {
            devs.emplace_back(new device_t());
            devs.back()->logical = (int)i;
            devs.back()->physical = ids[i];
        }
        configured = true;
    }
    int ndev() {
        configure();
        return (int)devs.size();
    }
    int device_of(const void* ptr) {
        configure();
        hipPointerAttribute_t at;
        if (!ptr || hipPointerGetAttributes(&at, ptr) != hipSuccess) {
            (void)hipGetLastError();
            return -1;
        }
        std::vector<int> match;
        for (auto& d : devs)
            if (d->physical == at.device) match.push_back(d->logical);
        if (match.empty()) return -1;
        return match[rr.fetch_add(1) % match.size()];
    }
};
extern runtime_t g_rt;

static void tu_kernel_attributes(int logical) {
    static std::mutex mu;
    static std::vector<char> done;
    std::lock_guard<std::mutex> lk(mu);
    if ((int)done.size() <= logical) done.resize(logical + 1, 0);
    if (done[logical]) return;
    HIP_TRY(hipFuncSetAttribute((const void*)scan_one_block_kernel, hipFuncAttributeMaxDynamicSharedMemorySize, (int)(SCAN_ONE_MAX * 4)));
#ifdef SV_TU_G1
    HIP_TRY(hipFuncSetAttribute((const void*)msm_accumulate_lazy_kernel<true>, hipFuncAttributeMaxDynamicSharedMemorySize, 128 * 1024));
#endif
#ifdef SV_TU_NTT
    HIP_TRY(hipFuncSetAttribute((const void*)ntt_pass_kernel_v2<false, ntt_arith_u>, hipFuncAttributeMaxDynamicSharedMemorySize, 96 * 1024));
    HIP_TRY(hipFuncSetAttribute((const void*)ntt_pass_kernel_v2<true, ntt_arith_u>, hipFuncAttributeMaxDynamicSharedMemorySize, 96 * 1024));
    HIP_TRY(hipFuncSetAttribute((const void*)ntt_pass_kernel_v2<true, ntt_arith_u, ntt_load_bounded>, hipFuncAttributeMaxDynamicSharedMemorySize, 96 * 1024));
    HIP_TRY(hipFuncSetAttribute((const void*)ntt_pass_kernel_v2<false, ntt_arith_u, ntt_load_product>, hipFuncAttributeMaxDynamicSharedMemorySize, 96 * 1024));
#endif
    done[logical] = 1;
}

static constexpr int SCOPE_AUX_MAX = 7;
struct scope_pending_t {
    hipEvent_t done;
    std::function<void()> finish;
    const void* tag;
};
struct thread_scope_t {
    lane_t* lane = nullptr;
    int prev_device = -1;
    unsigned flags = 0;
    lane_t* aux[SCOPE_AUX_MAX] = {};
    int naux = 0;
    unsigned aux_rr = 0;
    bool aux_exhausted = false;
    std::vector<scope_pending_t> pending;
    thread_scope_t() = default;
    thread_scope_t(const thread_scope_t&) = default;
    thread_scope_t& operator=(const thread_scope_t&) = default;
    ~thread_scope_t();
};
extern thread_local thread_scope_t g_tl_scope;
static thread_scope_t& tl_scope() { return g_tl_scope; }
static void scope_flush() {
    thread_scope_t& sc = tl_scope();
    if (!sc.lane) return;
    std::exception_ptr err;
    for (scope_pending_t& p : sc.pending) {
        try {
            HIP_TRY(hipEventSynchronize(p.done));
            p.finish();
        } catch (...) {
            if (!err) err = std::current_exception();
        }
    }
    sc.pending.clear();
    try {
        sc.lane->flush_scope();
        for (int i = 0; i < sc.naux; i++) HIP_TRY(hipStreamSynchronize(sc.aux[i]->stream));
    } catch (...) {
        if (!err) err = std::current_exception();
    }
    sc.lane->pin_used = 0;
    sc.lane->scope_events_used = 0;
    for (int i = 0; i < sc.naux; i++) sc.aux[i]->pin_used = 0, sc.aux[i]->scope_events_used = 0;
    if (err) std::rethrow_exception(err);
}
static void scope_collect(const void* tag) {
    thread_scope_t& sc = tl_scope();
    if (!sc.lane) return;
    std::exception_ptr err;
    if (tag) {
        auto ready = [](const scope_pending_t& p) {
            const hipError_t e = hipEventQuery(p.done);
            if (e == hipSuccess) return true;
            (void)hipGetLastError();
            return false;
        };
        auto wanted_ready = [&]() {
            for (const scope_pending_t& p : sc.pending)
                if (p.tag == tag && !ready(p)) return false;
            return true;
        };
        for (size_t i = 0; i < sc.pending.size() && !wanted_ready();) {
            if (sc.pending[i].tag != tag && ready(sc.pending[i])) {
                try {
                    sc.pending[i].finish();
                } catch (...) {
                    if (!err) err = std::current_exception();
                }
                sc.pending.erase(sc.pending.begin() + (ptrdiff_t)i);
            } else {
                i++;
            }
// ... 91 lines not shown
        for (size_t i = first_borrowed ? 1 : 0; i < lanes.size(); i++) lanes[i]->dev->give(lanes[i]);
        if (prev_device >= 0) (void)hipSetDevice(prev_device);
    }
};

inline ntt_ctx_t lane_t::ntt_ctx(hipStream_t st) { return ntt_ctx_t{st ? st : stream, &dev->tb, &dev->tw, &tw_leases}; }
inline void lane_t::begin_call() {
    phases.clear();
    events_used = 0;
}
inline void lane_t::phase_begin(const char* name) {
    if (!g_rt.profiling.load(std::memory_order_relaxed)) return;
    phase_rec r{name, new_event(), new_event(), 0.0};
    HIP_TRY(hipEventRecord(r.e0, stream));
    phases.push_back(r);
}
inline void lane_t::phase_end() {
    if (!g_rt.profiling.load(std::memory_order_relaxed) || phases.empty()) return;
    HIP_TRY(hipEventRecord(phases.back().e1, stream));
}
inline void lane_t::phase_host(const char* name, double ms) {
    if (!g_rt.profiling.load(std::memory_order_relaxed)) return;
    phases.push_back(phase_rec{name, nullptr, nullptr, ms});
}
static void ntt_tw_release(device_t* dev, std::vector<void*>& leases) { ntt_tw_release_entries(dev->tw, leases); }
inline void lane_t::flush_scope() {
    HIP_TRY(hipStreamSynchronize(stream));
    for (const deferred_out_t& d : deferred) memcpy(d.dst, pin2.as<uint8_t>() + d.off, d.bytes);
    deferred.clear();
    deferred_bytes = 0;
    if (!tw_leases.empty()) ntt_tw_release(dev, tw_leases);
    sv_drain_frees();
}
inline void lane_t::end_call() {
    if (in_scope) return;
    sv_drain_frees();
    if (!tw_leases.empty()) {
        HIP_TRY(hipStreamSynchronize(stream));
        ntt_tw_release(dev, tw_leases);
    }
    if (phases.empty()) return;
    HIP_TRY(hipStreamSynchronize(stream));
    std::vector<std::pair<std::string, double>> out;
    for (auto& r : phases) {
        if (r.e0) {
            float ms = 0;
            HIP_TRY(hipEventElapsedTime(&ms, r.e0, r.e1));
            r.ms = ms;
        }
        out.emplace_back(r.name, r.ms);
    }
    std::lock_guard<std::mutex> lk(g_rt.prof_mu);
    g_rt.last_phases.swap(out);
}

template <class Fn>
static void for_each_device(const std::vector<int>& devices, Fn fn) {
    if (devices.size() <= 1) {
        for (int d : devices) fn(d);
        return;
    }
    std::vector<std::thread> th;
    std::vector<std::exception_ptr> errs(devices.size());
    for (size_t i = 0; i < devices.size(); i++)
        th.emplace_back([&, i] {
            try {
                fn(devices[i]);
            } catch (...) {
                errs[i] = std::current_exception();
            }
        });
    for (auto& t : th) t.join();
    for (auto& e : errs)
        if (e) std::rethrow_exception(e);
}

struct msm_ticket_t;
template <class F>
struct bases_handle_t {
    std::vector<aff_mem_t<F>*> d;
    size_t n = 0;
    int tables = 1;
    int table_bits = 256;
    mutable std::mutex co_mu;
    mutable std::condition_variable co_cv;
    mutable std::deque<msm_ticket_t*> co_q;
    mutable int co_leaders = 0;
    void free_all() {
        int prev = 0;
        (void)hipGetDevice(&prev);
        for (size_t i = 0; i < d.size(); i++)
            if (d[i]) {
                (void)hipSetDevice(g_rt.devs[i]->physical);
                (void)hipFree(d[i]);
                d[i] = nullptr;
            }
        (void)hipSetDevice(prev);
    }
};
struct snarkvm_hip_bases : bases_handle_t<fq_t> {};

static const uint64_t FQ_R[6] = {202099033278250856ull,  5854854902718660529ull, 11492539364873682930ull,
                                 8885205928937022213ull, 5545221690922665192ull, 39800542322357402ull};
template <class F>
static void write_infinity(void* out) {
    const size_t fb = sizeof(typename F::mem_t);
    memset(out, 0, 3 * fb);
    memcpy((uint8_t*)out + fb, FQ_R, 48);
}

static constexpr int MSM_MAX_POS = 320;
template <class F>
struct msm_accum_t {
    xyzz_t<F> at[MSM_MAX_POS];
    bool used[MSM_MAX_POS];
    int top = -1;
    msm_accum_t() {
        for (int i = 0; i < MSM_MAX_POS; i++) used[i] = false;
    }
    void add(int pos, const xyzz_t<F>& p) {
        if (p.is_inf()) return;
        if (pos < 0 || pos >= MSM_MAX_POS) throw std::runtime_error("msm: bit position out of range");
        if (!used[pos]) {
            at[pos] = p;
            used[pos] = true;
        } else {
            at[pos].add(p);
        }
        if (pos > top) top = pos;
    }
    void finish(void* out) const {
        xyzz_t<F> t = xyzz_t<F>::inf();
        for (int p = top; p >= 0; p--) {
            t = t.dbl();
            if (used[p]) t.add(at[p]);
        }
        const jac_t<F> j = t.to_jacobian();
        uint32_t w[3 * F::MEM_WORDS];
        j.x.to_raw_words(w);
        j.y.to_raw_words(w + F::MEM_WORDS);
        j.z.to_raw_words(w + 2 * F::MEM_WORDS);
        memcpy(out, w, sizeof w);
    }
};
struct msm_pending_t {
    const void* planes = nullptr;
    int nplanes = 0;
    int tail_windows = 0, nbits = 0;
    int c = 0, m = 0;
    bool folded = false;
    int ninst = 0;
    bool lazy = false;
    int pos(int idx) const {
        const int tw = idx / nbits, j = idx % nbits;
        if (ninst) return (tw & 1) * m + j;
        return folded ? c * (tw >> 1) + (tw & 1) * m + j : c * tw + j;
    }
};
template <class F>
static constexpr size_t msm_point_bytes() {
    return sizeof(F) == sizeof(fq_t) && sizeof(xyzz_mem_t<fqz_t>) > sizeof(xyzz_mem_t<F>) ? sizeof(xyzz_mem_t<fqz_t>) : sizeof(xyzz_mem_t<F>);
}
template <class F>
static xyzz_t<F> msm_plane(const msm_pending_t& pd, int i) {
    if constexpr (sizeof(F) == sizeof(fq_t)) {
        if (pd.lazy) {
// ... 93 lines not shown
        const dim3 plane_grid((unsigned)g.nbits, (unsigned)g.tail_windows);
        hipLaunchKernelGGL((msm_bitplane_kernel<F, true>), plane_grid, dim3(plane_threads), 0, st, (const xyzz_mem_t<F>*)c.fold_sums.as<xyzz_mem_t<F>>(),
                           (const uint32_t*)nullptr, (const uint32_t*)nullptr, c.planes.as<xyzz_mem_t<F>>(), pl.nb, g.fold_m, g.fold_hb, hex, quads_planes, plane_flags);
        if constexpr (TAIL_FLAGGED<F>::value)
            hipLaunchKernelGGL((msm_bitplane_fix_kernel<F, true>), plane_grid, dim3(64), 0, st, (const xyzz_mem_t<F>*)c.fold_sums.as<xyzz_mem_t<F>>(), (const uint32_t*)nullptr,
                               (const uint32_t*)nullptr, c.planes.as<xyzz_mem_t<F>>(), pl.nb, g.fold_m, g.fold_hb, (const uint32_t*)plane_flags);
    } else {
        const dim3 plane_grid((unsigned)g.nbits, (unsigned)g.tail_windows);
        hipLaunchKernelGGL((msm_bitplane_kernel<F, false>), plane_grid, dim3(256), 0, st, sums, start, cnt, c.planes.as<xyzz_mem_t<F>>(), pl.nb, 0, 0, hex, 0, plane_flags);
        if constexpr (TAIL_FLAGGED<F>::value)
            hipLaunchKernelGGL((msm_bitplane_fix_kernel<F, false>), plane_grid, dim3(64), 0, st, sums, start, cnt, c.planes.as<xyzz_mem_t<F>>(), pl.nb, 0, 0,
                               (const uint32_t*)plane_flags);
    }
    HIP_TRY(hipGetLastError());
    HIP_TRY(hipMemcpyAsync(host_planes, c.planes.p, (size_t)pd.nplanes * sizeof(xyzz_mem_t<F>), hipMemcpyDeviceToHost, st));
}
struct msm_bucket_sink_t {
    void* acc = nullptr;
    uint32_t L = 1, slot = 0, nbt = 0;
    hipEvent_t after = nullptr, done = nullptr;
};
static int msm_trace_level() {
    static const int level = getenv("SNARKVM_HIP_TRACE") ? atoi(getenv("SNARKVM_HIP_TRACE")) : 0;
    return level;
}
struct msm_phases_t {
    lane_t& c;
    bool profile;
    int trace;
    size_t n;
    const char* cur = "";
    void begin(const char* name) {
        cur = name;
        if (trace >= 2) fprintf(stderr, "[snarkvm_hip] msm n=%zu: %s ...\n", n, name);
        if (profile) c.phase_begin(name);
    }
    void end() {
        if (profile) c.phase_end();
        if (trace >= 2) {
            const hipError_t e = hipStreamSynchronize(c.stream);
            fprintf(stderr, "[snarkvm_hip] msm n=%zu: %s done (%s)\n", n, cur, hipGetErrorString(e));
        }
    }
};
template <class T>
static void msm_reduce_and_tail(lane_t& c, const msm_plan_t& pl, const msm_tail_geom_t& tg, uint32_t nwin, uint32_t nbt, int rounds, size_t T0_max, size_t T1_max,
                                const msm_bucket_sink_t* sink, msm_pending_t& pd, void* host_planes, msm_phases_t& ph) {
    hipStream_t st = c.stream;
    ph.begin("msm_reduce_partials");
    uint32_t *cnt_in = c.cnt_a.as<uint32_t>(), *cnt_out = c.cnt_b.as<uint32_t>();
    uint32_t *start_in = c.start_a.as<uint32_t>(), *start_out = c.start_b.as<uint32_t>();
    xyzz_mem_t<T> *pin = c.part_a.as<xyzz_mem_t<T>>(), *pout = c.part_b.as<xyzz_mem_t<T>>();
    size_t T_in_max = T0_max;
    for (int r = 0; r < rounds; r++) {
        size_t T_out_max = T_in_max / pl.S2 + nbt + 1;
        if (T_out_max > T1_max) T_out_max = T1_max;
        hipLaunchKernelGGL(msm_alloc_kernel, dim3((nbt + 1 + 255) / 256), dim3(256), 0, st, cnt_in, cnt_out, nbt, pl.S2);
        exclusive_scan_u32(st, cnt_out, start_out, (size_t)nbt + 1, c.scan_tmp.as<uint32_t>());
        hipLaunchKernelGGL((msm_reduce_kernel<T>), dim3((unsigned)((T_out_max + 255) / 256)), dim3(256), 0, st, pin, start_in, cnt_in, start_out, pout, nbt,
                           pl.S2);
        std::swap(cnt_in, cnt_out);
        std::swap(start_in, start_out);
        std::swap(pin, pout);
        T_in_max = T_out_max;
    }
    ph.end();
    if (sink) {
        ph.begin("msm_bucket_merge");
        if (sink->after) HIP_TRY(hipStreamWaitEvent(st, sink->after, 0));
        hipLaunchKernelGGL((msm_bucket_merge_kernel<T>), dim3((nbt + 255) / 256), dim3(256), 0, st, (const xyzz_mem_t<T>*)pin, (const uint32_t*)start_in,
                           (const uint32_t*)cnt_in, (xyzz_mem_t<T>*)sink->acc, nbt, sink->L, sink->slot);
        if (sink->done) HIP_TRY(hipEventRecord(sink->done, st));
        ph.end();
        HIP_TRY(hipGetLastError());
        pd.nplanes = 0;
        return;
    }
    ph.begin("msm_bucket_reduce");
    msm_tail_launch<T>(c, pl, tg, nwin, nbt, pin, start_in, cnt_in, pd, host_planes);
    ph.end();
}
template <class F>
static void msm_launch_accumulate(lane_t& c, const msm_plan_t& pl, const aff_mem_t<F>* vbase, uint32_t* boffp, uint32_t nbt, size_t nthreads, bool one_wave,
                                  bool ltail) {
    hipStream_t st = c.stream;
#ifdef SV_BENCH
    static const uint32_t dbg_mask = getenv("SNARKVM_HIP_DEBUG_IDX_MASK") ? (uint32_t)strtoul(getenv("SNARKVM_HIP_DEBUG_IDX_MASK"), nullptr, 0) : 0xffffffffu;
#else
    constexpr uint32_t dbg_mask = 0xffffffffu;
#endif
    const size_t tmax = nthreads + nbt + 1;
    if constexpr (sizeof(F) == sizeof(fq_t)) {
        if (msm_lazy_on<F>()) {
            if (!ltail) c.part_raw.ensure(tmax * sizeof(g1_lazy_partial_t));
            g1_lazy_partial_t* raw_out = ltail ? c.part_a.as<g1_lazy_partial_t>() : c.part_raw.as<g1_lazy_partial_t>();
            hipLaunchKernelGGL((msm_accumulate_lazy_kernel<true>), dim3((unsigned)((nthreads + 255) / 256)), dim3(256), one_wave || tuning().acc_one_wg ? msm_acc_lds() : 0, st,
                               vbase, c.sorted.as<uint32_t>(), boffp, c.start_a.as<uint32_t>(), raw_out, nbt, pl.S, dbg_mask);
            if (!ltail)
                hipLaunchKernelGGL(g1_partials_to_exact_kernel, dim3((unsigned)((tmax + 255) / 256)), dim3(256), 0, st, (const g1_lazy_partial_t*)raw_out,
                                   c.part_a.as<g1_xyzz_mem_t>(), (const uint32_t*)c.start_a.as<uint32_t>(), nbt);
            return;
        }
    } else {
#ifndef SV_NO_G2
        if (msm_lazy_on<F>()) {
            c.part_raw.ensure(tmax * sizeof(g2_pair_partial_t));
            hipLaunchKernelGGL((msm_accumulate_pair2_kernel<false>), dim3((unsigned)((2 * nthreads + 255) / 256)), dim3(256), 0, st, vbase, c.sorted.as<uint32_t>(),
                               boffp, c.start_a.as<uint32_t>(), c.part_raw.as<g2_pair_partial_t>(), nbt, pl.S, dbg_mask);
            hipLaunchKernelGGL(g2_pair_partials_to_exact_kernel, dim3((unsigned)((8 * tmax + 255) / 256)), dim3(256), 0, st,
                               (const g2_pair_partial_t*)c.part_raw.as<g2_pair_partial_t>(), c.part_a.as<xyzz_mem_t<fq2_t>>(),
                               (const uint32_t*)c.start_a.as<uint32_t>(), nbt);
            return;
        }
#endif
    }
    if (one_wave)
        hipLaunchKernelGGL((msm_accumulate_seg_kernel<F, 1, true>), dim3((unsigned)((nthreads + 255) / 256)), dim3(256), 0, st, vbase, c.sorted.as<uint32_t>(), boffp,
                           c.start_a.as<uint32_t>(), c.part_a.as<xyzz_mem_t<F>>(), nbt, pl.S, dbg_mask);
    else
        hipLaunchKernelGGL((msm_accumulate_seg_kernel<F, 1, false>), dim3((unsigned)((nthreads + 255) / 256)), dim3(256), 0, st, vbase, c.sorted.as<uint32_t>(), boffp,
                           c.start_a.as<uint32_t>(), c.part_a.as<xyzz_mem_t<F>>(), nbt, pl.S, dbg_mask);
}
template <class F>
static size_t msm_plane_bytes() {
    return (size_t)MSM_MAX_POS * msm_point_bytes<F>();
}
template <class F>
struct msm_job_t {
    const aff_mem_t<F>* bases = nullptr;
    const aff_mem_t<F>* bases1 = nullptr;
    size_t n0 = 0;
    int tables = 1;
    size_t table_stride = 0;
    int table_bits = 0;
    const uint4* scalars = nullptr;
    size_t n = 0;
    int scalars_montgomery = 0;
    int window_bits = 0;
    void* host_planes = nullptr;
    bool profile = true;
    const msm_multi_t* multi = nullptr;
    const msm_bucket_sink_t* sink = nullptr;
    hipEvent_t scalars_read = nullptr;
};
template <class F>
struct msm_layout_t {
    msm_plan_t pl;
    bool wide;
    bool fused;
    bool ltail;
    bool single_round, prefetch_ok;
    uint32_t nwin, nbt;
    size_t E_max, T0_max, T1_max;
    const aff_mem_t<F>* vbase;
    msm_tail_geom_t tg;
    msm_radix_params_t rp;
    msm_digit_params_t dp;
    int LBL;
    uint32_t B1, nbins, nseg_last;
    size_t ncounts1, tiles1, tiles2_max;
};
template <class F>
static msm_layout_t<F> msm_layout(lane_t& c, const msm_job_t<F>& j, msm_pending_t& pd) {
    const msm_multi_t* mu = j.multi;
    const size_t n = j.n;
    size_t n0 = j.bases1 ? j.n0 : n;
    if (n0 > n) n0 = n;
    msm_layout_t<F> L{};
    if (n >= ((size_t)1 << 31)) throw hip_failure{hipErrorInvalidValue, "msm: npoints must be < 2^31", __LINE__};
    const msm_plan_t pl = L.pl = msm_make_plan(n, mu ? j.table_bits : j.window_bits, j.tables, j.table_bits);
    L.wide = pl.c > 16;
    if (mu && (L.wide || pl.W != 1 || pl.c < 12 || (size_t)pl.J * mu->hn >= ((size_t)1 << 31) || n != mu->npad || n % SORT_TILE))
        throw hip_failure{hipErrorInvalidValue, "msm: geometry not eligible for a fused multi-instance run", __LINE__};
    if ((size_t)pl.Wd * n >= ((size_t)1 << 32)) throw hip_failure{hipErrorInvalidValue, "msm: windows * npoints must be < 2^32", __LINE__};
    if ((size_t)pl.J * n >= ((size_t)1 << 31)) throw hip_failure{hipErrorInvalidValue, "msm: tables * npoints must be < 2^31", __LINE__};
    const aff_mem_t<F>* vb1 = j.bases1 ? j.bases1 : j.bases;
    L.vbase = mu ? j.bases : (vb1 < j.bases ? vb1 : j.bases);
    if (!mu) {
        const size_t top0 = (size_t)(j.bases - L.vbase) + n0, top1 = (size_t)(vb1 - L.vbase) + (n - n0);
        if ((size_t)(pl.J - 1) * j.table_stride + (top0 > top1 ? top0 : top1) >= ((size_t)1 << 31))
            throw hip_failure{hipErrorInvalidValue, "msm: base slots must be addressable in 31 bits (tables * registered points < 2^31)", __LINE__};
    }
    const size_t E_max = L.E_max = (size_t)pl.Wd * n;
    const uint32_t nwin = L.nwin = mu ? mu->K : (uint32_t)pl.W;
    const uint32_t nbt = L.nbt = nwin * pl.nb;

    c.scan_tmp.ensure((scan_tmp_elems((size_t)nbt + 1)) * 4);
    c.boff.ensure(((size_t)nbt + 2) * 4);
    c.cnt_a.ensure(((size_t)nbt + 1) * 4);
    c.cnt_b.ensure(((size_t)nbt + 1) * 4);
    c.start_a.ensure(((size_t)nbt + 1) * 4);
    c.start_b.ensure(((size_t)nbt + 1) * 4);
    const size_t slack = (size_t)nbt / 32 + 64;
    L.T0_max = E_max / pl.S + nbt + 1 + slack;
    L.T1_max = L.T0_max / pl.S2 + nbt + 1 + slack;
    pd.lazy = L.ltail = msm_lazy_tail_on<F>();
    c.part_a.ensure(L.T0_max * msm_partial_bytes<F>());
    c.part_b.ensure(L.T1_max * msm_partial_bytes<F>());
    L.tg = msm_tail_geometry(pl, nwin, pd, mu ? (int)mu->K : 0);
    if (mu && (size_t)pd.nplanes > mu->plane_capacity) throw hip_failure{hipErrorInvalidValue, "msm: plane staging of the fused group too small", __LINE__};
    if (j.sink && (mu || j.sink->nbt != nbt)) throw hip_failure{hipErrorInvalidValue, "msm: bucket sink does not match the plan", __LINE__};
    c.planes.ensure((size_t)pd.nplanes * msm_partial_bytes<F>());

    L.fused = !mu && L.wide && tuning().fused && pl.c <= 22 && pl.Wd <= FUSED_MAX_ROWS;
    memcpy(L.dp.bias, pl.bias, sizeof L.dp.bias);
    L.dp.c = pl.c;
    L.dp.W = pl.Wd;
    L.dp.n = n;
    L.dp.montgomery = j.scalars_montgomery;
    L.single_round = mu || (size_t)pl.Wd * n <= ((size_t)1 << 22);
    L.prefetch_ok = (size_t)pl.Wd * n <= ((size_t)1 << 22);

    msm_radix_params_t& rp = L.rp;
// ... 124 lines not shown
    if (j.multi)
        hipLaunchKernelGGL(radix_bin_layout_multi_kernel, dim3((L.nbins + 1 + 255) / 256), dim3(256), 0, st, off1, counts1, L.ncounts1,
                           c.rbinstart.as<uint32_t>(), L.nbins, L.rp);
    else
        hipLaunchKernelGGL(radix_bin_layout_kernel, dim3((L.nbins + 1 + 255) / 256), dim3(256), 0, st, off1, counts1, L.ncounts1, c.rbinstart.as<uint32_t>(),
                           L.nbins, L.rp.TPW);
    ph.end();
}
static void msm_tile_segments(lane_t& c, const uint32_t* seg_start, uint32_t nseg) {
    hipLaunchKernelGGL(radix_bin_tiles_kernel, dim3((nseg + 1 + 255) / 256), dim3(256), 0, c.stream, seg_start, c.rntiles.as<uint32_t>(), nseg);
    exclusive_scan_u32(c.stream, c.rntiles.as<uint32_t>(), c.rtstart.as<uint32_t>(), (size_t)nseg + 1, c.scan_tmp.as<uint32_t>());
}
static void msm_colscan(lane_t& c, uint32_t* sizes, uint32_t nsegs, int bits, uint32_t* dmax) {
    if (nsegs <= 4096)
        hipLaunchKernelGGL(radix_colscan2_seg_kernel, dim3(nsegs), dim3(1024), 0, c.stream, c.rcounts2.as<uint32_t>(), c.roff2.as<uint32_t>(),
                           c.rtstart.as<uint32_t>(), sizes, nsegs, bits, dmax);
    else
        hipLaunchKernelGGL(radix_colscan2_kernel, dim3(((nsegs << bits) + 1 + 255) / 256), dim3(256), 0, c.stream, c.rcounts2.as<uint32_t>(),
                           c.roff2.as<uint32_t>(), c.rtstart.as<uint32_t>(), sizes, nsegs, bits, dmax);
}
template <class F>
static void msm_stage_sort_rest(lane_t& c, const msm_layout_t<F>& L, msm_phases_t& ph) {
    hipStream_t st = c.stream;
    const size_t E_max = L.E_max;
    const uint32_t nbt = L.nbt;
    uint32_t* bsize = c.rbsize.as<uint32_t>();
    uint32_t* d_max = bsize + nbt + 1;
    uint32_t* boffp = c.boff.as<uint32_t>();
    const uint32_t* seg_start = c.rbinstart.as<uint32_t>();
    uint32_t nseg = L.nbins;
    const uint32_t* v_in = c.rv1.as<uint32_t>();
    if (L.wide) {
        ph.begin("msm_sort_level2");
        const uint32_t ngroups = nseg << 7;
        const size_t tmax = E_max / SORT_TILE + nseg + 1;
        c.rv2.ensure(E_max * 4);
        c.rl2.ensure(E_max);
        c.rmid_size.ensure(((size_t)ngroups + 3) * 4);
        c.rmid_boff.ensure(((size_t)ngroups + 3) * 4);
        c.scan_tmp.ensure(scan_tmp_elems((size_t)ngroups + 2) * 4);
        uint32_t* msize = c.rmid_size.as<uint32_t>();
        uint32_t* mboff = c.rmid_boff.as<uint32_t>();
        msm_tile_segments(c, seg_start, nseg);
        hipLaunchKernelGGL((radix_hist2_kernel<uint16_t>), dim3((unsigned)tmax), dim3(SORT_THREADS), 0, st, c.rl1.as<uint16_t>(), seg_start,
                           c.rtstart.as<uint32_t>(), c.rcounts2.as<uint32_t>(), nseg, 7, 7);
        HIP_TRY(hipMemsetAsync(msize + ngroups + 1, 0, 4, st));
        msm_colscan(c, msize, nseg, 7, msize + ngroups + 1);
        exclusive_scan_u32(st, msize, mboff, (size_t)ngroups + 1, c.scan_tmp.as<uint32_t>());
        hipLaunchKernelGGL((radix_scatter2_kernel<uint16_t, uint8_t>), dim3((unsigned)tmax), dim3(SORT_THREADS), 0, st, v_in, c.rl1.as<uint16_t>(),
                           seg_start, c.rtstart.as<uint32_t>(), c.rcounts2.as<uint32_t>(), c.roff2.as<uint32_t>(), mboff, c.rv2.as<uint32_t>(),
                           c.rl2.as<uint8_t>(), nseg, 7, 7, (uint32_t)tuning().xcd);
        ph.end();
        seg_start = mboff;
        nseg = ngroups;
        v_in = c.rv2.as<uint32_t>();
    }
    ph.begin(L.wide ? "msm_sort_level3" : "msm_sort_level2");
    msm_tile_segments(c, seg_start, nseg);
    const uint8_t* rem_last = L.wide ? c.rl2.as<uint8_t>() : c.rl1.as<uint8_t>();
    hipLaunchKernelGGL((radix_hist2_kernel<uint8_t>), dim3((unsigned)L.tiles2_max), dim3(SORT_THREADS), 0, st, rem_last, seg_start,
                       c.rtstart.as<uint32_t>(), c.rcounts2.as<uint32_t>(), nseg, L.LBL, 0);
    HIP_TRY(hipMemsetAsync(d_max, 0, 4, st));
    msm_colscan(c, bsize, nseg, L.LBL, d_max);
    exclusive_scan_u32(st, bsize, boffp, (size_t)nbt + 1, c.scan_tmp.as<uint32_t>());
    hipLaunchKernelGGL((radix_scatter2_kernel<uint8_t, uint8_t>), dim3((unsigned)L.tiles2_max), dim3(SORT_THREADS), 0, st, v_in, rem_last, seg_start,
                       c.rtstart.as<uint32_t>(), c.rcounts2.as<uint32_t>(), c.roff2.as<uint32_t>(), boffp, c.sorted.as<uint32_t>(),
                       (uint8_t*)nullptr, nseg, L.LBL, 0, (uint32_t)tuning().xcd);
    ph.end();
}
template <class F>
static int msm_stage_accumulate(lane_t& c, const msm_layout_t<F>& L, const msm_job_t<F>& j, msm_phases_t& ph) {
    hipStream_t st = c.stream;
    const msm_multi_t* mu = j.multi;
    const uint32_t nbt = L.nbt;
    uint32_t* boffp = c.boff.as<uint32_t>();
    int rounds = 0;
    ph.begin("msm_accumulate");
    const int env_rounds = tuning().reduce_rounds;
    if (!L.single_round) rounds = env_rounds < 0 ? 0 : (env_rounds > 8 ? 8 : env_rounds);
    if (mu && tuning().fuse_reduce > 0) rounds = tuning().fuse_reduce > 4 ? 4 : tuning().fuse_reduce;
    if (mu && tuning().fuse_reduce < 0) rounds = mu->K >= 8 ? 1 : 0;
    hipLaunchKernelGGL(msm_alloc_seg_kernel, dim3((nbt + 1 + 255) / 256), dim3(256), 0, st, boffp, c.cnt_a.as<uint32_t>(), nbt, L.pl.S);
    exclusive_scan_u32(st, c.cnt_a.as<uint32_t>(), c.start_a.as<uint32_t>(), (size_t)nbt + 1, c.scan_tmp.as<uint32_t>());
    msm_launch_accumulate<F>(c, L.pl, L.vbase, boffp, nbt, (L.E_max + L.pl.S - 1) / L.pl.S, L.single_round && L.prefetch_ok, L.ltail);
    ph.end();
    return rounds;
}
template <class T>
struct msm_field_tag {
    using type = T;
};
template <class F, class Fn>
static void msm_on_tail_field(bool lazy, Fn&& fn) {
    if constexpr (sizeof(F) == sizeof(fq_t)) {
        if (lazy) return fn(msm_field_tag<fqz_t>{});
    }
    fn(msm_field_tag<F>{});
}
template <class F>
static msm_pending_t msm_run(lane_t& c, const msm_job_t<F>& j) {
    msm_pending_t pd;
    pd.planes = j.host_planes;
    if (j.n == 0) return pd;
    msm_phases_t ph{c, j.profile, msm_trace_level(), j.n};
    const msm_layout_t<F> L = msm_layout(c, j, pd);
    if (!L.fused) msm_stage_digits(c, L, j, ph);
    msm_stage_level1(c, L, j, ph);
    msm_stage_sort_rest(c, L, ph);
    const int rounds = msm_stage_accumulate(c, L, j, ph);
    msm_on_tail_field<F>(L.ltail, [&](auto t) {
        msm_reduce_and_tail<typename decltype(t)::type>(c, L.pl, L.tg, L.nwin, L.nbt, rounds, L.T0_max, L.T1_max, j.sink, pd, j.host_planes, ph);
    });
    return pd;
}
template <class F>
static msm_pending_t msm_tail_from_sink(lane_t& c, const msm_job_t<F>& j, const msm_bucket_sink_t& sink) {
    msm_pending_t pd;
    pd.planes = j.host_planes;
    const msm_plan_t pl = msm_make_plan(j.n, j.window_bits, j.tables, j.table_bits);
    const uint32_t nwin = (uint32_t)pl.W, nbt = nwin * pl.nb;
    if (nbt != sink.nbt) throw hip_failure{hipErrorInvalidValue, "msm: bucket sink does not match the plan", __LINE__};
    const msm_tail_geom_t tg = msm_tail_geometry(pl, nwin, pd, 0);
    c.start_a.ensure(((size_t)nbt + 1) * 4);
    c.cnt_a.ensure(((size_t)nbt + 1) * 4);
    hipLaunchKernelGGL(msm_sink_lists_kernel, dim3((nbt + 1 + 255) / 256), dim3(256), 0, c.stream, c.start_a.as<uint32_t>(), c.cnt_a.as<uint32_t>(), nbt, sink.L);
    pd.lazy = msm_lazy_tail_on<F>();
    c.phase_begin("msm_bucket_reduce");
    msm_on_tail_field<F>(pd.lazy, [&](auto t) {
        using T = typename decltype(t)::type;
        msm_tail_launch<T>(c, pl, tg, nwin, nbt, (const xyzz_mem_t<T>*)sink.acc, c.start_a.as<uint32_t>(), c.cnt_a.as<uint32_t>(), pd, j.host_planes);
    });
    c.phase_end();
    return pd;
}
template <class F>
static void msm_run_sync(lane_t& c, const msm_job_t<F>& j, void* out) {
    if (c.in_scope && c.pin_used) scope_flush();
    c.pin.ensure(msm_plane_bytes<F>());
    msm_job_t<F> staged = j;
    staged.host_planes = c.pin.p;
    const msm_pending_t pd = msm_run<F>(c, staged);
    HIP_TRY(hipStreamSynchronize(c.stream));
    const double t0 = host_now_ms();
    msm_accum_t<F>* acc = new msm_accum_t<F>();
    std::unique_ptr<msm_accum_t<F>> hold(acc);
    msm_collect<F>(*acc, pd);
    acc->finish(out);
    c.phase_host("msm_host_finish", host_now_ms() - t0);
}

template <class F>
static bool msm_lazy_on() {
    return sizeof(F) == sizeof(fq_t) ? tuning().lazy != 0 : tuning().lazy2 != 0;
}
template <class F>
static void convert_bases(lane_t& c, const uint8_t* d_in, size_t stride, size_t n, aff_mem_t<F>* d_out, hipStream_t st = nullptr, bool for_msm = false) {
    if (!n) return;
    const int form406 = for_msm && msm_lazy_on<F>() ? 1 : 0;
    hipLaunchKernelGGL((convert_bases_kernel<F>), dim3((unsigned)((n + 255) / 256)), dim3(256), 0, st ? st : c.stream, d_in, stride, n, d_out, form406);
    HIP_TRY(hipGetLastError());
}
static void bases_to_lazy_form(lane_t& c, g1_aff_mem_t* d, size_t slots) {
    if (!slots || !msm_lazy_on<fq_t>()) return;
    hipLaunchKernelGGL(g1_bases_to_form406_kernel, dim3((unsigned)((slots + 255) / 256)), dim3(256), 0, c.stream, d, slots);
    HIP_TRY(hipGetLastError());
}
#ifndef SV_NO_G2
static void bases_to_lazy_form(lane_t& c, aff_mem_t<fq2_t>* d, size_t slots) {
    if (!slots || !msm_lazy_on<fq2_t>()) return;
    hipLaunchKernelGGL(g2_bases_to_form406_kernel, dim3((unsigned)((slots + 255) / 256)), dim3(256), 0, c.stream, d, slots);
    HIP_TRY(hipGetLastError());
}
#endif

template <class F>
static void precompute_tables_run(lane_t& c, aff_mem_t<F>* d, size_t n, int tables, int table_bits) {
    if (tables <= 1 || !n) return;
    int run = (int)(n >> 16);
    run = run < 1 ? 1 : (run > PRE_RUN ? PRE_RUN : run);
    const size_t slab = n < PRE_SLAB ? n : PRE_SLAB;
    c.gen_pts.ensure(4 * slab * sizeof(typename F::mem_t));
    for (int j = 1; j < tables; j++)
        for (size_t lo = 0; lo < n; lo += PRE_SLAB) {
            const size_t cnt = n - lo < PRE_SLAB ? n - lo : PRE_SLAB;
            const size_t threads = (cnt + run - 1) / run;
            hipLaunchKernelGGL((precompute_table_kernel<F>), dim3((unsigned)((threads + 255) / 256)), dim3(256), 0, c.stream, d + (size_t)(j - 1) * n + lo,
                               d + (size_t)j * n + lo, cnt, table_bits, run, (typename F::mem_t*)c.gen_pts.p);
        }
    HIP_TRY(hipGetLastError());
}

static int batch_lanes(size_t npoints) {
    const int env = tuning().lanes;
    int l = env > 0 ? env : (npoints >= ((size_t)1 << 20) ? 3 : 8);
    return l < 1 ? 1 : (l > device_t::LANES ? device_t::LANES : l);
}
static constexpr size_t MSM_SPLIT_MIN = (size_t)1 << 18;
static size_t msm_chunk_pairs() {
    const int lg = tuning().msm_chunk_lg;
    return (size_t)1 << (lg < 16 ? 16 : (lg > 30 ? 30 : lg));
}
static size_t msm_scalar_chunk_pairs() {
    const int lg = tuning().scalar_chunk_lg;
    return (size_t)1 << (lg < 18 ? 18 : lg > 30 ? 30 : lg);
}

template <class Upload, class Compute>
static void lane_ring_run(lane_guard& lg, size_t count, Upload&& upload, Compute&& compute, int trace, double t_begin) {
    const size_t L = lg.lanes.size();
    const int phys = lg.lanes[0]->dev->physical;
    std::mutex mu;
    std::condition_variable cv;
    std::vector<char> uploaded(count, 0), enqueued(count, 0);
    std::vector<hipEvent_t> up(count), used(count);
    for (size_t j = 0; j < count; j++) {
        up[j] = lg.lanes[j % L]->new_event();
        used[j] = lg.lanes[j % L]->new_event();
    }
    std::exception_ptr up_err, cp_err;
    std::thread uploader([&] {
        try {
            HIP_TRY(hipSetDevice(phys));
            for (size_t j = 0; j < count; j++) {
                lane_t& c = *lg.lanes[j % L];
                if (j >= L) {
                    char state;
                    {
                        std::unique_lock<std::mutex> lk(mu);
                        cv.wait(lk, [&] { return enqueued[j - L] != 0; });
                        state = enqueued[j - L];
                    }
                    if (state == 2) break;
                    HIP_TRY(hipEventSynchronize(used[j - L]));
                }
                const double t0 = host_now_ms();
                upload(j, c.alt);
                HIP_TRY(hipEventRecord(up[j], c.alt));
                if (trace) fprintf(stderr, "[snarkvm_hip] chunk %zu dev %d lane %d: uploaded t+%.2f .. t+%.2f ms\n", j, c.dev->logical, c.index, t0 - t_begin, host_now_ms() - t_begin);
                {
                    std::lock_guard<std::mutex> lk(mu);
                    uploaded[j] = 1;
                }
                cv.notify_all();
            }
        } catch (...) {
            up_err = std::current_exception();
            std::lock_guard<std::mutex> lk(mu);
            for (auto& u : uploaded) u = 2;
            cv.notify_all();
// ... 119 lines not shown
        auto chunk_lo = [&](size_t j) { return bound[mine[j]]; };
        auto chunk_cnt = [&](size_t j) { return bound[mine[j] + 1] - bound[mine[j]]; };
        auto upload = [&](size_t j, hipStream_t st) {
            lane_t& c = *lg.lanes[j % L];
            uint8_t* raw = c.bases_tmp.template as<uint8_t>() + aff_bytes;
            HIP_TRY(hipMemcpyAsync(raw, (const uint8_t*)points + chunk_lo(j) * stride, chunk_cnt(j) * stride, hipMemcpyHostToDevice, st));
            HIP_TRY(hipMemcpyAsync(c.scalars_tmp.p, (const uint8_t*)scalars + chunk_lo(j) * 32, chunk_cnt(j) * 32, hipMemcpyHostToDevice, st));
        };
        auto compute = [&](size_t j, bool prof) {
            lane_t& c = *lg.lanes[j % L];
            uint8_t* raw = c.bases_tmp.template as<uint8_t>() + aff_bytes;
            if (prof) c.phase_begin("msm_convert_bases");
            convert_bases<F>(c, raw, stride, chunk_cnt(j), c.bases_tmp.template as<aff_mem_t<F>>(), nullptr, true);
            if (prof) c.phase_end();
            msm_bucket_sink_t mine_sink = sink;
            mine_sink.slot = (uint32_t)(j % L);
            msm_job_t<F> job;
            job.bases = c.bases_tmp.template as<aff_mem_t<F>>();
            job.scalars = c.scalars_tmp.template as<uint4>();
            job.n = chunk_cnt(j);
            job.window_bits = chunk_c;
            job.host_planes = c.pin.template as<uint8_t>() + (use_sink ? 0 : slot * (j / L));
            job.profile = prof;
            job.sink = use_sink ? &mine_sink : nullptr;
            const msm_pending_t pd = msm_run<F>(c, job);
            if (!use_sink) pend[j] = pd;
        };
        if (mine.size() == 1) {
            lane_t& c = *lg.lanes[0];
            c.phase_begin("msm_h2d");
            upload(0, c.stream);
            c.phase_end();
            compute(0, true);
        } else {
            lane_ring_run(lg, mine.size(), upload, [&](size_t j) { compute(j, false); }, trace, t_begin);
        }
        if (use_sink) {
            lane_t& c0 = *lg.lanes[0];
            for (int l = 1; l < L; l++) {
                hipEvent_t e = lg.lanes[l]->new_event();
                HIP_TRY(hipEventRecord(e, lg.lanes[l]->stream));
                HIP_TRY(hipStreamWaitEvent(c0.stream, e, 0));
            }
            msm_job_t<F> tail;
            tail.n = max_cnt;
            tail.window_bits = chunk_c;
            tail.host_planes = c0.pin.p;
            pend[0] = msm_tail_from_sink<F>(c0, tail, sink);
        }
        for (int l = 0; l < L; l++) {
            HIP_TRY(hipStreamSynchronize(lg.lanes[l]->alt));
            HIP_TRY(hipStreamSynchronize(lg.lanes[l]->stream));
        }
        const double t_sync = host_now_ms();
        {
            std::lock_guard<std::mutex> lk(acc_mu);
            for (auto& pd : pend) msm_collect<F>(*acc, pd);
        }
        if (trace) fprintf(stderr, "[snarkvm_hip] all chunks done at t+%.2f ms, planes collected in %.2f ms\n", t_sync - t_begin, host_now_ms() - t_sync);
        for (int l = 0; l < L; l++) lg.lanes[l]->end_call();
    });
    acc->finish(out);
}

static constexpr size_t MSM_FUSE_MAX_PAIRS = (size_t)1 << 18;
static constexpr size_t MSM_FUSE_MAX_ENTRIES = (size_t)1 << 26;
static bool msm_fuse_enabled() {
    return tuning().fuse_batch != 0;
}
static size_t msm_fuse_max_k() {
    const int k = tuning().fuse_max_k;
    return (size_t)(k < 2 ? 2 : (k > 256 ? 256 : k));
}
struct msm_req_t {
    size_t off0 = 0, n0 = 0, off1 = 0, n1 = 0;
    const void* scalars = nullptr;
    void* out = nullptr;
};
template <class F>
static msm_job_t<F> msm_handle_job(const bases_handle_t<F>& h, int dev, const msm_req_t& r) {
    msm_job_t<F> j;
    j.bases = h.d[dev] + r.off0;
    j.bases1 = r.n1 ? h.d[dev] + r.off1 : nullptr;
    j.n0 = r.n0;
    j.tables = h.tables;
    j.table_stride = h.n;
    j.table_bits = h.table_bits;
    j.n = r.n0 + r.n1;
    return j;
}
template <class Fn>
static void host_parallel_for(size_t n, int max_threads, Fn fn) {
    size_t T = n / 4;
    if (T > (size_t)max_threads) T = (size_t)max_threads;
    if (T <= 1) {
        for (size_t i = 0; i < n; i++) fn(i);
        return;
    }
    std::atomic<size_t> next{0};
    std::vector<std::exception_ptr> errs(T);
    auto work = [&](size_t t) {
        try {
            for (size_t i; (i = next.fetch_add(1)) < n;) fn(i);
        } catch (...) {
            errs[t] = std::current_exception();
        }
    };
    std::vector<std::thread> th;
    for (size_t t = 1; t < T; t++) th.emplace_back(work, t);
    work(0);
    for (auto& x : th) x.join();
    for (auto& e : errs)
        if (e) std::rethrow_exception(e);
}
template <class F>
static bool msm_handle_fusable(const bases_handle_t<F>& h, int window_bits) {
    if (!msm_fuse_enabled() || h.tables <= 1 || h.table_bits < 12 || h.table_bits > 16 || (window_bits != 0 && window_bits != h.table_bits) ||
        (size_t)h.tables * h.n >= ((size_t)1 << 31) || h.n >= ((size_t)1 << 31))
        return false;
    const msm_plan_t pl = msm_make_plan(SORT_TILE, h.table_bits, h.tables, h.table_bits);
    return pl.W == 1 && pl.c == h.table_bits;
}
template <class F>
static size_t msm_fuse_planes(const bases_handle_t<F>& h) {
    return 2 * ((size_t)h.table_bits / 2 + 1);
}
static size_t msm_padded(size_t n) { return (n + SORT_TILE - 1) / SORT_TILE * SORT_TILE; }
template <class F>
static std::vector<std::vector<size_t>> msm_make_jobs(const bases_handle_t<F>& h, const msm_req_t* req, const std::vector<size_t>& mine, bool fusable_handle) {
    std::vector<std::vector<size_t>> jobs;
    std::vector<size_t> group;
    size_t group_entries = 0;
    auto flush = [&] {
        if (!group.empty()) jobs.push_back(group);
        group.clear();
        group_entries = 0;
    };
    for (size_t k : mine) {
        const size_t tot = req[k].n0 + req[k].n1;
        const bool small = fusable_handle && tot > 0 && tot <= MSM_FUSE_MAX_PAIRS;
        if (!small) {
            jobs.push_back({k});
            continue;
        }
        const size_t e = msm_padded(tot) * (size_t)h.tables;
        if (!group.empty() && (group.size() >= msm_fuse_max_k() || group_entries + e > MSM_FUSE_MAX_ENTRIES)) flush();
        group.push_back(k);
        group_entries += e;
    }
    flush();
    return jobs;
}
template <class F>
static void msm_job_staging(const bases_handle_t<F>& h, const std::vector<size_t>& job, size_t& plane_bytes, size_t& table_bytes) {
    const size_t K = job.size();
    plane_bytes = K > 1 ? K * msm_fuse_planes(h) * msm_point_bytes<F>() : msm_plane_bytes<F>();
    table_bytes = K > 1 ? ((K + 1) * sizeof(msm_inst_t) + 255) / 256 * 256 : 0;
}
template <class F>
static msm_pending_t msm_enqueue_job(lane_t& c, const bases_handle_t<F>& h, int dev, const msm_req_t* req, const std::vector<size_t>& job, uint8_t* host_planes,
                                     msm_inst_t* tab, int scalars_on_device, int scalars_montgomery, int window_bits, hipEvent_t scalars_read = nullptr) {
    if (job.size() == 1) {
        const msm_req_t& r = req[job[0]];
        const size_t n = r.n0 + r.n1;
        const uint4* d_sc = (const uint4*)r.scalars;
        if (!scalars_on_device && n) {
// ... 440 lines not shown
```

snarkvm_amd/csrc/tuning.hip.h:

```cpp
#pragma once
#include <stdio.h>
#include <stdlib.h>
#include <string.h>

namespace sv {

struct tuning_t {
    int lazy = 1, lazy2 = 1, fused = 1;
    long acc_lds = 96 * 1024;
    int acc_one_wg = 0, reduce_rounds = 1, fuse_batch = 1, fuse_max_k = 64, fuse_reduce = -1, coalesce = 1, coalesce_us = 40, lanes = 0;
    int msm_chunk_lg = 20, scalar_chunk_lg = 22, taper = 1, ring_lanes = 3, seg = 0, seg2 = 0, fold_l = 0, scan1 = 1;
    int ntt_min_tiles = 256, ntt_full_tw = 1, ntt_fold = 1, ntt_batch = 1;
    int xcd = 1, fold_threads2 = 128, coalesce_slots = 2, ramp = 3, scalar_geo = 4, lazy_tail = 1, horner2 = 1, hex2 = 1, group_quad = 1, tail_quads = 13, fold_small2 = 256, fold_mid = 128;

    bool set(const char* key, long v) {
#define SV_TUNE_KEY(name)                  \
    if (!strcmp(key, #name)) {             \
        name = (decltype(name))v;          \
        return true;                       \
    }
        SV_TUNE_KEY(lazy) SV_TUNE_KEY(lazy2) SV_TUNE_KEY(fused) SV_TUNE_KEY(acc_lds)
        SV_TUNE_KEY(acc_one_wg) SV_TUNE_KEY(reduce_rounds) SV_TUNE_KEY(fuse_batch) SV_TUNE_KEY(fuse_max_k) SV_TUNE_KEY(fuse_reduce) SV_TUNE_KEY(coalesce)
        SV_TUNE_KEY(coalesce_us) SV_TUNE_KEY(lanes) SV_TUNE_KEY(msm_chunk_lg) SV_TUNE_KEY(scalar_chunk_lg) SV_TUNE_KEY(taper) SV_TUNE_KEY(ring_lanes) SV_TUNE_KEY(seg) SV_TUNE_KEY(seg2)
        SV_TUNE_KEY(fold_l) SV_TUNE_KEY(scan1) SV_TUNE_KEY(ntt_min_tiles) SV_TUNE_KEY(ntt_full_tw) SV_TUNE_KEY(ntt_fold)
        SV_TUNE_KEY(ntt_batch) SV_TUNE_KEY(xcd) SV_TUNE_KEY(fold_threads2) SV_TUNE_KEY(coalesce_slots) SV_TUNE_KEY(ramp) SV_TUNE_KEY(scalar_geo) SV_TUNE_KEY(lazy_tail) SV_TUNE_KEY(horner2) SV_TUNE_KEY(hex2) SV_TUNE_KEY(group_quad) SV_TUNE_KEY(tail_quads) SV_TUNE_KEY(fold_small2) SV_TUNE_KEY(fold_mid)
#undef SV_TUNE_KEY
        return false;
    }
    void parse(const char* s) {
        while (s && *s) {
            while (*s == ',' || *s == ' ') s++;
            const char* eq = strchr(s, '=');
            const char* end = strchr(s, ',');
            if (!end) end = s + strlen(s);
            if (!*s) break;
            char key[32] = {0};
            if (!eq || eq > end || (size_t)(eq - s) >= sizeof key) {
                fprintf(stderr, "[snarkvm_hip] SNARKVM_HIP_TUNING: malformed item at \"%s\" (ignored)\n", s);
            } else {
                memcpy(key, s, (size_t)(eq - s));
                char* num_end = nullptr;
                const long v = strtol(eq + 1, &num_end, 0);
                if (num_end == eq + 1 || !set(key, v)) fprintf(stderr, "[snarkvm_hip] SNARKVM_HIP_TUNING: unknown key or bad value \"%s\" (ignored)\n", key);
            }
            s = end;
        }
    }
    void clamp() {
        auto fix = [](const char* key, auto& v, long lo, long hi) {
            if ((long)v < lo || (long)v > hi) {
                const long was = (long)v;
                v = (decltype(v + 0))((long)v < lo ? lo : hi);
                fprintf(stderr, "[snarkvm_hip] SNARKVM_HIP_TUNING: %s=%ld is out of range [%ld, %ld]; using %ld\n", key, was, lo, hi, (long)v);
            }
        };
        fix("coalesce_slots", coalesce_slots, 1, 8);
        fix("coalesce_us", coalesce_us, 0, 100000);
        fix("fuse_max_k", fuse_max_k, 2, 256);
        fix("fuse_reduce", fuse_reduce, -1, 4);
        fix("reduce_rounds", reduce_rounds, 0, 8);
        fix("lanes", lanes, 0, 8);
        fix("ring_lanes", ring_lanes, 2, 8);
        fix("ntt_min_tiles", ntt_min_tiles, 1, 1 << 20);
        fix("acc_lds", acc_lds, 0, 160 * 1024);
        fix("msm_chunk_lg", msm_chunk_lg, 16, 30);
        fix("scalar_chunk_lg", scalar_chunk_lg, 18, 30);
        fix("ramp", ramp, 0, 6);
        fix("scalar_geo", scalar_geo, 0, 16);
        fix("seg", seg, 0, 4096);
        fix("seg2", seg2, 0, 256);
        fix("fold_l", fold_l, 0, 64);
    }
};
inline const tuning_t& tuning() {
    static const tuning_t t = [] {
        tuning_t v;
        v.parse(getenv("SNARKVM_HIP_TUNING"));
        v.clamp();
        return v;
    }();
    return t;
}

}
```

snarkvm_amd/msm.py:

```python
import ctypes

import numpy as np

from . import _lib, plugin
from .layout import G1_AFFINE, G1_PROJECTIVE


class VariableBase:
    @staticmethod
    def msm(bases, scalars):
        return plugin.msm(bases, scalars)


class RegisteredBases:

    def __init__(self, bases=None, device_ptr=None, npoints=None, tables=1, window_bits=0):
        L = _lib.lib()
        self._h = ctypes.c_void_p()
        self.tables = int(tables)
        self.window_bits = int(window_bits)
        if device_ptr is not None:
            self.n = int(npoints)
            src, on_device = ctypes.c_void_p(device_ptr), 1
        else:
            bases = np.ascontiguousarray(bases, dtype=G1_AFFINE).reshape(-1)
            self.n = bases.shape[0]
            src, on_device = ctypes.c_void_p(bases.ctypes.data), 0
        if self.window_bits:
            err = L.snarkvm_hip_register_bases_windowed(ctypes.byref(self._h), src, ctypes.c_size_t(self.n), ctypes.c_size_t(G1_AFFINE.itemsize),
                                                        ctypes.c_int(on_device), ctypes.c_int(self.tables), ctypes.c_int(self.window_bits))
        else:
            err = L.snarkvm_hip_register_bases_tables(ctypes.byref(self._h), src, ctypes.c_size_t(self.n), ctypes.c_size_t(G1_AFFINE.itemsize),
                                                      ctypes.c_int(on_device), ctypes.c_int(self.tables))
        _lib.check(err)

    @classmethod
    def from_serialized(cls, data, npoints, compressed=False, validate=False, tables=1):
        from . import serialize

        self = cls.__new__(cls)
        self.tables = int(tables)
        self.window_bits = 0
        self.n = int(npoints)
        self._h = serialize.register_bases_serialized(data, npoints, compressed, validate, tables)
        return self

    def msm(self, scalars=None, offset=0, device_ptr=None, npoints=None, window_bits=0):
        L = _lib.lib()
        out = np.zeros(1, dtype=G1_PROJECTIVE)
        if device_ptr is not None:
            n = int(npoints)
            err = L.snarkvm_hip_msm_registered(ctypes.c_void_p(out.ctypes.data), self._h, ctypes.c_size_t(offset), ctypes.c_size_t(n),
                                               ctypes.c_void_p(device_ptr), ctypes.c_int(1), ctypes.c_int(window_bits))
        else:
            scalars = np.ascontiguousarray(scalars, dtype=np.uint64).reshape(-1, 4)
            n = scalars.shape[0]
            err = L.snarkvm_hip_msm_registered(ctypes.c_void_p(out.ctypes.data), self._h, ctypes.c_size_t(offset), ctypes.c_size_t(n),
                                               ctypes.c_void_p(scalars.ctypes.data), ctypes.c_int(0), ctypes.c_int(window_bits))
        _lib.check(err)
        return out

    def msm_batch(self, scalars_list=None, offsets=None, device_ptrs=None, npoints=None, window_bits=0, montgomery=False):
        L = _lib.lib()
        if device_ptrs is not None:
            count = len(device_ptrs)
            ns = [int(v) for v in npoints]
            ptrs = [int(p) for p in device_ptrs]
            on_dev = 1
            keep = None
        else:
            keep = [np.ascontiguousarray(s, dtype=np.uint64).reshape(-1, 4) for s in scalars_list]
            count = len(keep)
            ns = [k.shape[0] for k in keep]
            ptrs = [k.ctypes.data for k in keep]
            on_dev = 0
        offs = [0] * count if offsets is None else [int(o) for o in offsets]
        out = np.zeros(count, dtype=G1_PROJECTIVE)
        c_offs = (ctypes.c_size_t * max(1, count))(*offs)
        c_ns = (ctypes.c_size_t * max(1, count))(*ns)
        c_ptrs = (ctypes.c_void_p * max(1, count))(*ptrs)
        _lib.check(L.snarkvm_hip_msm_registered_batch(ctypes.c_void_p(out.ctypes.data), self._h, ctypes.c_size_t(count), c_offs, c_ns, c_ptrs,
                                                      ctypes.c_int(on_dev), ctypes.c_int(1 if montgomery else 0), ctypes.c_int(window_bits)))
        return out

    def close(self):
        if self._h:
            _lib.lib().snarkvm_hip_free_bases(self._h)
            self._h = ctypes.c_void_p()

    def __del__(self):
        try:
            self.close()
        except Exception:
            pass


def msm_g2(bases, scalars):
    from .layout import G2_AFFINE, G2_PROJECTIVE

    bases = np.ascontiguousarray(bases, dtype=G2_AFFINE).reshape(-1)
    scalars = np.ascontiguousarray(scalars, dtype=np.uint64).reshape(-1, 4)
    n = scalars.shape[0]
    if n > bases.shape[0]:
        raise ValueError(f"length mismatch {bases.shape[0]} points < {n} scalars")
    out = np.zeros(1, dtype=G2_PROJECTIVE)
    err = _lib.lib().snarkvm_hip_msm_g2(ctypes.c_void_p(out.ctypes.data), ctypes.c_void_p(bases.ctypes.data), ctypes.c_size_t(n),
                                        ctypes.c_void_p(scalars.ctypes.data), ctypes.c_size_t(G2_AFFINE.itemsize))
    _lib.check(err)
    return out


class RegisteredBasesG2:

    def __init__(self, bases, tables=16, window_bits=0):
        from .layout import G2_AFFINE

        bases = np.ascontiguousarray(bases, dtype=G2_AFFINE).reshape(-1)
        self.n = bases.shape[0]
        self._h = ctypes.c_void_p()
        _lib.check(_lib.lib().snarkvm_hip_register_bases_g2(ctypes.byref(self._h), ctypes.c_void_p(bases.ctypes.data), ctypes.c_size_t(self.n),
                                                           ctypes.c_size_t(G2_AFFINE.itemsize), ctypes.c_int(int(tables)), ctypes.c_int(int(window_bits))))

    def msm(self, scalars=None, offset=0, window_bits=0, device_ptr=None, npoints=None):
        from .layout import G2_PROJECTIVE

        out = np.zeros(1, dtype=G2_PROJECTIVE)
        if device_ptr is not None:
            _lib.check(_lib.lib().snarkvm_hip_msm_g2_registered(ctypes.c_void_p(out.ctypes.data), self._h, ctypes.c_size_t(offset),
                                                               ctypes.c_size_t(int(npoints)), ctypes.c_void_p(device_ptr), ctypes.c_int(1),
                                                               ctypes.c_int(window_bits)))
            return out
        scalars = np.ascontiguousarray(scalars, dtype=np.uint64).reshape(-1, 4)
        _lib.check(_lib.lib().snarkvm_hip_msm_g2_registered(ctypes.c_void_p(out.ctypes.data), self._h, ctypes.c_size_t(offset),
                                                           ctypes.c_size_t(scalars.shape[0]), ctypes.c_void_p(scalars.ctypes.data), ctypes.c_int(0),
                                                           ctypes.c_int(window_bits)))
        return out

    def msm_batch(self, scalars_list=None, offsets=None, device_ptrs=None, npoints=None, window_bits=0):
        from .layout import G2_PROJECTIVE

        if device_ptrs is not None:
            count, ns, ptrs, on_dev, keep = len(device_ptrs), [int(v) for v in npoints], [int(p) for p in device_ptrs], 1, None
        else:
            keep = [np.ascontiguousarray(s, dtype=np.uint64).reshape(-1, 4) for s in scalars_list]
            count, ns, ptrs, on_dev = len(keep), [k.shape[0] for k in keep], [k.ctypes.data for k in keep], 0
        offs = [0] * count if offsets is None else [int(o) for o in offsets]
        out = np.zeros(count, dtype=G2_PROJECTIVE)
        c_offs = (ctypes.c_size_t * max(1, count))(*offs)
        c_ns = (ctypes.c_size_t * max(1, count))(*ns)
        c_ptrs = (ctypes.c_void_p * max(1, count))(*ptrs)
        _lib.check(_lib.lib().snarkvm_hip_msm_g2_registered_batch(ctypes.c_void_p(out.ctypes.data), self._h, ctypes.c_size_t(count), c_offs, c_ns, c_ptrs,
                                                                 ctypes.c_int(on_dev), ctypes.c_int(window_bits)))
        return out

    def close(self):
        if self._h:
            _lib.lib().snarkvm_hip_free_bases_g2(self._h)
            self._h = ctypes.c_void_p()

    def __del__(self):
        try:
            self.close()
        except Exception:
            pass


# ... 19 lines not shown
```

Before: 565.2 million pairs/s.

## Accumulate G1 MSM buckets in twisted Edwards coordinates with precomputed base slots

At registration, the G1 bases are checked for subgroup membership and converted into a twisted Edwards representation (three precomputed operands per point, 192-byte slots). The bucket accumulation then runs a new Edwards mixed-add kernel that reads these slots, and its partials are converted back to XYZZ form for the reduction. Mixed addition on Edwards curves is cheaper than short-Weierstrass XYZZ addition and needs no special cases. In exchange the slots are larger, which raises memory traffic and HBM footprint, and registration pays for a subgroup check and a conversion pass. The Edwards path is enabled by default, with a fallback to the old lazy form when the subgroup check fails.

Result: slower. 547.9 million pairs/s (-3.1%).

```diff
diff --git a/include/snarkvm_hip.h b/include/snarkvm_hip.h
--- a/include/snarkvm_hip.h
+++ b/include/snarkvm_hip.h
@@ -68,6 +68,7 @@
 RustError snarkvm_hip_register_bases_windowed(snarkvm_hip_bases_t **handle, const void *points, size_t npoints,
                                               size_t ffi_affine_sz, int on_device, int tables, int window_bits);
 void snarkvm_hip_free_bases(snarkvm_hip_bases_t *handle);
+int snarkvm_hip_bases_form(const snarkvm_hip_bases_t *handle);
 
 RustError snarkvm_hip_register_bases_serialized(snarkvm_hip_bases_t **handle, const void *bytes, size_t npoints,
                                                 int compressed, int validate, int tables);
@@ -159,6 +160,7 @@
 int snarkvm_hip_selftest_msm_plan(size_t n, int window_bits, int tables, int table_bits, uint32_t *out);
 int snarkvm_hip_selftest_g1_finish(const void *planes_projective, const int32_t *pos, size_t n, void *out);
 int snarkvm_hip_selftest_fq_lazy(uint64_t seed, int iters);
+int snarkvm_hip_selftest_g1_edwards(int op, const void *in, size_t n, const void *aux, size_t m, void *out);
 int snarkvm_hip_selftest_g1_lazy_tail(uint64_t seed, int iters);
 int snarkvm_hip_selftest_fq2_pair(const void *points, size_t npoints, uint64_t seed, int iters);
 int snarkvm_hip_selftest_g2_hex(const void *points, size_t npoints, uint64_t seed, int iters);
diff --git a/rust/snarkvm-algorithms-hip/src/sys.rs b/rust/snarkvm-algorithms-hip/src/sys.rs
--- a/rust/snarkvm-algorithms-hip/src/sys.rs
+++ b/rust/snarkvm-algorithms-hip/src/sys.rs
@@ -46,6 +46,7 @@
     pub fn snarkvm_hip_register_bases_tables(handle: *mut *mut snarkvm_hip_bases_t, points: *const c_void, npoints: usize, ffi_affine_sz: usize, on_device: i32, tables: i32) -> Error;
     pub fn snarkvm_hip_register_bases_windowed(handle: *mut *mut snarkvm_hip_bases_t, points: *const c_void, npoints: usize, ffi_affine_sz: usize, on_device: i32, tables: i32, window_bits: i32) -> Error;
     pub fn snarkvm_hip_free_bases(handle: *mut snarkvm_hip_bases_t);
+    pub fn snarkvm_hip_bases_form(handle: *const snarkvm_hip_bases_t) -> i32;
     pub fn snarkvm_hip_register_bases_serialized(handle: *mut *mut snarkvm_hip_bases_t, bytes: *const c_void, npoints: usize, compressed: i32, validate: i32, tables: i32) -> Error;
     pub fn snarkvm_hip_g1_deserialize(out_affine: *mut c_void, bytes: *const c_void, n: usize, compressed: i32, validate: i32) -> Error;
     pub fn snarkvm_hip_g1_serialize(out_bytes: *mut c_void, affine: *const c_void, n: usize, ffi_affine_sz: usize, compressed: i32) -> Error;
@@ -92,6 +93,7 @@
     pub fn snarkvm_hip_selftest_msm_plan(n: usize, window_bits: i32, tables: i32, table_bits: i32, out: *mut u32) -> i32;
     pub fn snarkvm_hip_selftest_g1_finish(planes_projective: *const c_void, pos: *const i32, n: usize, out: *mut c_void) -> i32;
     pub fn snarkvm_hip_selftest_fq_lazy(seed: u64, iters: i32) -> i32;
+    pub fn snarkvm_hip_selftest_g1_edwards(op: i32, in_: *const c_void, n: usize, aux: *const c_void, m: usize, out: *mut c_void) -> i32;
     pub fn snarkvm_hip_selftest_g1_lazy_tail(seed: u64, iters: i32) -> i32;
     pub fn snarkvm_hip_selftest_fq2_pair(points: *const c_void, npoints: usize, seed: u64, iters: i32) -> i32;
     pub fn snarkvm_hip_selftest_g2_hex(points: *const c_void, npoints: usize, seed: u64, iters: i32) -> i32;
diff --git a/snarkvm_amd/_lib.py b/snarkvm_amd/_lib.py
--- a/snarkvm_amd/_lib.py
+++ b/snarkvm_amd/_lib.py
@@ -9,7 +9,7 @@
     "snarkvm_hip_device_count", "snarkvm_hip_batch_lanes", "snarkvm_hip_set_device", "snarkvm_hip_set_devices", "snarkvm_hip_num_devices",
     "snarkvm_hip_malloc", "snarkvm_hip_free", "snarkvm_hip_memcpy_h2d", "snarkvm_hip_memcpy_d2h", "snarkvm_hip_memcpy_d2d", "snarkvm_hip_memset", "snarkvm_hip_ntt_device", "snarkvm_hip_ntt_device_batch", "snarkvm_hip_polymul_device",
     "snarkvm_hip_scope_begin", "snarkvm_hip_scope_end", "snarkvm_hip_scope_begin_ex", "snarkvm_hip_scope_collect", "snarkvm_hip_scope_set_flags", "snarkvm_hip_scope_stream", "snarkvm_hip_alloc_stats",
-    "snarkvm_hip_register_bases", "snarkvm_hip_register_bases_tables", "snarkvm_hip_register_bases_windowed", "snarkvm_hip_free_bases", "snarkvm_hip_msm_registered", "snarkvm_hip_msm_g2",
+    "snarkvm_hip_register_bases", "snarkvm_hip_register_bases_tables", "snarkvm_hip_register_bases_windowed", "snarkvm_hip_free_bases", "snarkvm_hip_bases_form", "snarkvm_hip_msm_registered", "snarkvm_hip_msm_g2",
     "snarkvm_hip_msm_registered_ex", "snarkvm_hip_msm_registered_batch", "snarkvm_hip_msm_registered_batch_ex", "snarkvm_hip_g1_to_affine",
     "snarkvm_hip_fr_mul_device", "snarkvm_hip_fr_convert_device", "snarkvm_hip_g1_generate_bases_device",
     "snarkvm_hip_fr_vec_op", "snarkvm_hip_fr_divide_by_linear", "snarkvm_hip_fr_batch_inversion_and_mul",
@@ -21,7 +21,7 @@
     "snarkvm_hip_g1_fixed_base_msm", "snarkvm_hip_g1_group_ntt",
     "snarkvm_hip_set_profiling", "snarkvm_hip_get_phase_count", "snarkvm_hip_get_phase_name",
     "snarkvm_hip_get_phase_ms", "snarkvm_hip_synchronize", "snarkvm_hip_coalescer_stats",
-    "snarkvm_hip_selftest_field", "snarkvm_hip_selftest_g1_msm_naive", "snarkvm_hip_selftest_msm_plan", "snarkvm_hip_selftest_g1_finish", "snarkvm_hip_selftest_fq_lazy", "snarkvm_hip_selftest_g1_lazy_tail", "snarkvm_hip_selftest_ntt_plan", "snarkvm_hip_selftest_ntt_twiddle", "snarkvm_hip_selftest_ntt_index", "snarkvm_hip_selftest_ntt_host", "snarkvm_hip_selftest_fq2_pair", "snarkvm_hip_selftest_g2_hex", "snarkvm_hip_selftest_fr_lincomb", "snarkvm_hip_devtest_field", "snarkvm_hip_devtest_g2_tail_repeat",
+    "snarkvm_hip_selftest_field", "snarkvm_hip_selftest_g1_msm_naive", "snarkvm_hip_selftest_msm_plan", "snarkvm_hip_selftest_g1_finish", "snarkvm_hip_selftest_fq_lazy", "snarkvm_hip_selftest_g1_edwards", "snarkvm_hip_selftest_g1_lazy_tail", "snarkvm_hip_selftest_ntt_plan", "snarkvm_hip_selftest_ntt_twiddle", "snarkvm_hip_selftest_ntt_index", "snarkvm_hip_selftest_ntt_host", "snarkvm_hip_selftest_fq2_pair", "snarkvm_hip_selftest_g2_hex", "snarkvm_hip_selftest_fr_lincomb", "snarkvm_hip_devtest_field", "snarkvm_hip_devtest_g2_tail_repeat",
 ]
 
 
@@ -71,6 +71,10 @@
         L.snarkvm_hip_num_devices.restype = ctypes.c_int
         L.snarkvm_hip_selftest_g1_finish.restype = ctypes.c_int
         L.snarkvm_hip_selftest_fq_lazy.restype = ctypes.c_int
+        L.snarkvm_hip_selftest_g1_edwards.restype = ctypes.c_int
+        L.snarkvm_hip_selftest_g1_edwards.argtypes = [ctypes.c_int, ctypes.c_void_p, ctypes.c_size_t, ctypes.c_void_p, ctypes.c_size_t, ctypes.c_void_p]
+        L.snarkvm_hip_bases_form.restype = ctypes.c_int
+        L.snarkvm_hip_bases_form.argtypes = [ctypes.c_void_p]
         L.snarkvm_hip_selftest_g1_lazy_tail.restype = ctypes.c_int
         for name in ("snarkvm_hip_selftest_ntt_plan", "snarkvm_hip_selftest_ntt_twiddle", "snarkvm_hip_selftest_ntt_index", "snarkvm_hip_selftest_ntt_host"):
             getattr(L, name).restype = ctypes.c_int
diff --git a/snarkvm_amd/csrc/api.hip b/snarkvm_amd/csrc/api.hip
--- a/snarkvm_amd/csrc/api.hip
+++ b/snarkvm_amd/csrc/api.hip
@@ -259,6 +259,9 @@
     return r;
 }
 
+}
+int sv_finish_g1_tables(lane_t& c, g1_aff_mem_t** d, size_t npoints, int tables) { return g1_tables_to_msm_form<0>(c, d, npoints, tables); }
+extern "C" {
 static void precompute_tables(lane_t& c, snarkvm_hip_bases* h, g1_aff_mem_t* d) { precompute_tables_run<fq_t>(c, d, h->n, h->tables, h->table_bits); }
 static void register_bases_impl(snarkvm_hip_bases_t** handle, const void* points, size_t npoints, size_t ffi_affine_sz, int on_device, int tables,
                                 int table_bits) {
@@ -274,6 +277,7 @@
     h->table_bits = table_bits ? table_bits : 256 / tables;
     h->d.assign(nd, nullptr);
     const size_t bytes = (size_t)tables * npoints * sizeof(g1_aff_mem_t);
+    std::vector<int> forms(nd, 0);
     try {
         if (npoints) {
             const int owner = on_device ? device_for(points, 1) : -1;
@@ -289,20 +293,25 @@
                 }
                 convert_bases<fq_t>(c, src, ffi_affine_sz, npoints, h->d[dev]);
                 precompute_tables(c, h.get(), h->d[dev]);
-                bases_to_lazy_form(c, h->d[dev], (size_t)tables * npoints);
+                forms[dev] = sv_finish_g1_tables(c, &h->d[dev], npoints, tables);
                 HIP_TRY(hipStreamSynchronize(c.stream));
             };
             std::vector<int> all;
             for (int d = 0; d < nd; d++) all.push_back(d);
             if (!on_device) {
                 for_each_device(all, build);
+                for (int d = 1; d < nd; d++)
+                    if (forms[d] != forms[0]) throw hip_failure{hipErrorUnknown, "register_bases: the replicas disagree on the form of the tables", __LINE__};
+                h->form = forms[0];
             } else {
                 build(owner);
+                h->form = forms[owner];
+                const size_t copy_bytes = g1_table_bytes(h->form, (size_t)tables * npoints);
                 for (int d = 0; d < nd; d++) {
                     if (d == owner) continue;
                     lane_guard lg(d);
-                    HIP_TRY(hipMalloc((void**)&h->d[d], bytes));
-                    HIP_TRY(hipMemcpyPeerAsync(h->d[d], g_rt.devs[d]->physical, h->d[owner], g_rt.devs[owner]->physical, bytes, lg.c().stream));
+                    HIP_TRY(hipMalloc((void**)&h->d[d], copy_bytes));
+                    HIP_TRY(hipMemcpyPeerAsync(h->d[d], g_rt.devs[d]->physical, h->d[owner], g_rt.devs[owner]->physical, copy_bytes, lg.c().stream));
                     HIP_TRY(hipStreamSynchronize(lg.c().stream));
                 }
             }
@@ -331,6 +340,7 @@
     register_bases_impl(handle, points, npoints, ffi_affine_sz, on_device, tables, window_bits);
     API_CATCH
 }
+int snarkvm_hip_bases_form(const snarkvm_hip_bases_t* h) { return h ? h->form : 0; }
 void snarkvm_hip_free_bases(snarkvm_hip_bases_t* h) {
     if (!h) return;
     h->free_all();
@@ -1112,6 +1122,74 @@
     }
     return 0;
 }
+int snarkvm_hip_selftest_g1_edwards(int op, const void* in, size_t n, const void* aux, size_t m, void* out) {
+    if (!out || (n && !in)) return -1;
+    uint32_t* o = (uint32_t*)out;
+    if (op == 0) {
+        const uint32_t* tabs[5] = {G1Ed::S, G1Ed::C, G1Ed::F, G1Ed::CF, G1Ed::K2D};
+        for (int t = 0; t < 5; t++)
+            for (int i = 0; i < 13; i++) o[13 * t + i] = tabs[t][i];
+        for (int i = 0; i < 8; i++) o[65 + i] = G1Ed::ORDER[i];
+        return 0;
+    }
+    std::vector<g1_aff_mem_t> pts(n ? n : 1);
+    for (size_t i = 0; i < n; i++) {
+        const uint32_t* src = (const uint32_t*)((const uint8_t*)in + i * 104);
+        g1_aff_t a = g1_aff_t::inf();
+        if (!(src[24] & 0xff)) a = {fq_t::unpack(src).from_mem_mont(), fq_t::unpack(src + 12).from_mem_mont()};
+        store_aff<fq_t>(&pts[i], a);
+    }
+    if (op == 4) {
+        for (size_t i = 0; i < n; i++) ((uint8_t*)out)[i] = g1_in_subgroup(g1_load_aff(&pts[i])) ? 1 : 0;
+        return 0;
+    }
+    std::vector<g1_ed_slot_t> slots(n ? n : 1);
+    for (size_t lo = 0; lo < n; lo += G1_ED_RUN) g1_ed_convert_run(&pts[lo], &slots[lo], n - lo < (size_t)G1_ED_RUN ? (int)(n - lo) : G1_ED_RUN);
+    if (op == 1) {
+        for (size_t i = 0; i < n; i++) memcpy(o + 39 * i, slots[i].w, 39 * 4);
+        return 0;
+    }
+    if (op != 2 && op != 3) return -2;
+    if (m && !aux) return -1;
+    const uint32_t* steps = (const uint32_t*)aux;
+    ed_lazy_t acc = ed_lazy_t::identity();
+    fql_t pat[4];
+    for (int i = 0; i < 13; i++) pat[0].v[i] = i < 12 ? (int32_t)fql_t::MASK : -1;
+    for (int i = 0; i < 13; i++) pat[1].v[i] = -FqL::MOD[i];
+    pat[1].v[0] += 1;
+    pat[1] = pat[1].normalized();
+    for (int i = 0; i < 13; i++) pat[2].v[i] = i == 12 ? -(FqL::MOD[12] / 2) : ((i & 1) ? (int32_t)fql_t::MASK : 0);
+    pat[3] = fql_t::zero();
+    pat[3].v[0] = 1;
+    for (size_t k = 0; k < m; k++) {
+        const uint32_t st = steps[k];
+        const size_t idx = st & 0x3fffffffu;
+        if (idx >= n) return -3;
+        if (st & 0x40000000u) acc = ed_lazy_t::identity();
+        if (op == 3) {
+            fql_t* cs[4] = {&acc.X, &acc.Y, &acc.Z, &acc.T};
+            const fq_t cur = cs[k & 3]->to_exact();
+            if (!cur.is_zero()) {
+                const fql_t& want = pat[(k >> 2) & 3];
+                const fql_t l = fql_t::from_exact(want.to_exact() * cur.inverse());
+                const int which = (int)(k & 3);
+                for (int c4 = 0; c4 < 4; c4++)
+                    if (c4 != which) *cs[c4] = fql_t::mul(*cs[c4], l);
+                *cs[which] = want;
+            }
+        }
+        fql_t a0, a1, a2;
+        g1_ed_raw_t::load(&slots[idx]).operands(a0, a1, a2);
+        acc.madd(a0, a1, a2, (st >> 31) != 0);
+        alignas(16) g1_lazy_partial_t raw;
+        acc.store_raw(&raw);
+        const g1_jac_t j = ed_lazy_t::exact_xyzz_from_raw(&raw).to_jacobian();
+        j.x.to_mem_mont().pack(o + 36 * k);
+        j.y.to_mem_mont().pack(o + 36 * k + 12);
+        j.z.to_mem_mont().pack(o + 36 * k + 24);
+    }
+    return 0;
+}
 int snarkvm_hip_selftest_g1_lazy_tail(uint64_t seed, int iters) {
     uint32_t xw[12], yw[12];
     memcpy(xw, G1_GEN_X, 48);
diff --git a/snarkvm_amd/csrc/api_serde.hip b/snarkvm_amd/csrc/api_serde.hip
--- a/snarkvm_amd/csrc/api_serde.hip
+++ b/snarkvm_amd/csrc/api_serde.hip
@@ -2,6 +2,7 @@
 
 snarkvm_hip_bases* sv_new_bases_handle(size_t npoints, int tables, int table_bits);
 void sv_precompute_tables(lane_t& c, snarkvm_hip_bases* h, g1_aff_mem_t* d);
+int sv_finish_g1_tables(lane_t& c, g1_aff_mem_t** d, size_t npoints, int tables);
 
 static uint32_t g1_deserialize_run(lane_t& c, const void* bytes, size_t n, int compressed, int validate, g1_aff_mem_t* d_native, uint8_t* d_rust) {
     const size_t psz = compressed ? 48 : 96;
@@ -30,15 +31,19 @@
         try {
             std::vector<int> all;
             for (int d = 0; d < g_rt.ndev(); d++) all.push_back(d);
+            std::vector<int> forms(all.size(), 0);
             for_each_device(all, [&](int dev) {
                 lane_guard lg(dev);
                 lane_t& c = lg.c();
                 HIP_TRY(hipMalloc((void**)&h->d[dev], (size_t)tables * npoints * sizeof(g1_aff_mem_t)));
                 serde_throw_on_status(g1_deserialize_run(c, bytes, npoints, compressed, validate, h->d[dev], nullptr), "register_bases_serialized");
                 sv_precompute_tables(c, h.get(), h->d[dev]);
-                bases_to_lazy_form(c, h->d[dev], (size_t)tables * npoints);
+                forms[dev] = sv_finish_g1_tables(c, &h->d[dev], npoints, tables);
                 HIP_TRY(hipStreamSynchronize(c.stream));
             });
+            for (size_t d = 1; d < forms.size(); d++)
+                if (forms[d] != forms[0]) throw hip_failure{hipErrorUnknown, "register_bases_serialized: the replicas disagree on the form of the tables", __LINE__};
+            h->form = forms[0];
         } catch (...) {
             h->free_all();
             throw;
diff --git a/snarkvm_amd/csrc/g1_edwards.hip.h b/snarkvm_amd/csrc/g1_edwards.hip.h
--- /dev/null
+++ b/snarkvm_amd/csrc/g1_edwards.hip.h
@@ -0,0 +1,174 @@
+#pragma once
+#include "ffl.hip.h"
+
+namespace sv {
+
+struct G1Ed {
+    static constexpr uint32_t S[13] = {0x08449ac2, 0x16bc6341, 0x1f27346e, 0x003fa706, 0x16341794, 0x0e03035e, 0x1f0a2ed9, 0x0c4c0908, 0x1a0645ff, 0x0dd41749, 0x078fb647, 0x1b5db1c4, 0x1660c39d};
+    static constexpr uint32_t C[13] = {0x18cdd044, 0x13a929c3, 0x1d759d09, 0x1349e454, 0x199c43da, 0x07d95012, 0x00a594f1, 0x0823ddd6, 0x17de8c4a, 0x02b23149, 0x13919ff6, 0x1304d1a1, 0x0d5b0216};
+    static constexpr uint32_t F[13] = {0x18d0ec00, 0x19d5ac0b, 0x099a00af, 0x14f3163d, 0x15201f1a, 0x185e2df4, 0x10000b58, 0x16cc24d5, 0x0cfaac7e, 0x1feb43c4, 0x0f6e64c6, 0x1143d6d9, 0x182ac132};
+    static constexpr uint32_t CF[13] = {0x04353bcb, 0x00c919fa, 0x1e46cd5a, 0x0ca605e1, 0x051d56cd, 0x180681eb, 0x0e770a1f, 0x164e2080, 0x061a7557, 0x1ccd125e, 0x08f96217, 0x1f09f0df, 0x0057ca06};
+    static constexpr uint32_t K2D[13] = {0x114806b1, 0x04ef4e0d, 0x07df1bf4, 0x01a7dedd, 0x07626a98, 0x061c00c8, 0x1b3f730c, 0x037d439d, 0x1c957daa, 0x096f1594, 0x098747ae, 0x19dba77f, 0x03dbbc1f};
+    static constexpr uint32_t ORDER[8] = {0x00000001u, 0x0a118000u, 0xd0000001u, 0x59aa76feu, 0x5c37b001u, 0x60b44d1eu, 0x9a2ca556u, 0x12ab655eu};
+};
+
+#ifndef SV_ED_SLOT_BYTES
+#define SV_ED_SLOT_BYTES 192
+#endif
+struct alignas(64) g1_ed_slot_t {
+    uint32_t w[SV_ED_SLOT_BYTES / 4];
+    static constexpr int QUADS = 10;
+    SV_HD void store(const fq_t& a0, const fq_t& a1, const fq_t& a2) {
+        uint32_t t[40];
+#pragma unroll
+        for (int i = 0; i < 13; i++) t[i] = a0.v[i], t[13 + i] = a1.v[i], t[26 + i] = a2.v[i];
+        t[39] = 0;
+        uint4* q = (uint4*)w;
+#pragma unroll
+        for (int i = 0; i < QUADS; i++) q[i] = make_uint4(t[4 * i], t[4 * i + 1], t[4 * i + 2], t[4 * i + 3]);
+#pragma unroll
+        for (int i = QUADS; i < SV_ED_SLOT_BYTES / 16; i++) q[i] = make_uint4(0, 0, 0, 0);
+    }
+};
+static_assert(sizeof(g1_ed_slot_t) == SV_ED_SLOT_BYTES && SV_ED_SLOT_BYTES % 64 == 0 && SV_ED_SLOT_BYTES >= 160, "Edwards base slot");
+struct g1_ed_raw_t {
+    uint4 q[g1_ed_slot_t::QUADS];
+    SV_HD static g1_ed_raw_t load(const g1_ed_slot_t* p) {
+        g1_ed_raw_t r;
+        const uint4* s = (const uint4*)p->w;
+#pragma unroll
+        for (int i = 0; i < g1_ed_slot_t::QUADS; i++) r.q[i] = s[i];
+        return r;
+    }
+    SV_HD void operands(fql_t& a0, fql_t& a1, fql_t& a2) const {
+        uint32_t t[40];
+#pragma unroll
+        for (int i = 0; i < g1_ed_slot_t::QUADS; i++) t[4 * i] = q[i].x, t[4 * i + 1] = q[i].y, t[4 * i + 2] = q[i].z, t[4 * i + 3] = q[i].w;
+#pragma unroll
+        for (int i = 0; i < 13; i++) a0.v[i] = (int32_t)t[i], a1.v[i] = (int32_t)t[13 + i], a2.v[i] = (int32_t)t[26 + i];
+        SV_OPAQUE_13(a0.v);
+        SV_OPAQUE_13(a1.v);
+        SV_OPAQUE_13(a2.v);
+    }
+};
+
+struct ed_lazy_t {
+    fql_t X, Y, Z, T;
+
+    SV_HD static fql_t table(const uint32_t* t) {
+        fql_t r;
+#pragma unroll
+        for (int i = 0; i < fql_t::N; i++) r.v[i] = (int32_t)t[i];
+        return r;
+    }
+    SV_HD static ed_lazy_t identity() {
+        ed_lazy_t r;
+        r.X = r.T = fql_t::zero();
+        r.Y = r.Z = xyzz_lazy_t::one();
+        return r;
+    }
+    SV_HD void madd(const fql_t& a0_in, const fql_t& a1_in, const fql_t& a2, bool negate) {
+        fql_t a0, a1;
+#pragma unroll
+        for (int i = 0; i < fql_t::N; i++) a0.v[i] = negate ? a1_in.v[i] : a0_in.v[i], a1.v[i] = negate ? a0_in.v[i] : a1_in.v[i];
+        const fql_t A = fql_t::mul(Y - X, a0);
+        const fql_t B = fql_t::mul((Y + X).normalized(), a1);
+        const fql_t C = fql_t::mul(T, a2).negate_if(negate);
+        const fql_t D = Z + Z;
+        const fql_t E = B - A;
+        const fql_t F = (D - C).normalized();
+        const fql_t G = (D + C).normalized();
+        const fql_t H = (B + A).normalized();
+        X = fql_t::mul(E, F);
+        Y = fql_t::mul(G, H);
+        T = fql_t::mul(E, H);
+        Z = fql_t::mul(F, G);
+    }
+    SV_HD void store_raw(g1_lazy_partial_t* p) const {
+        uint4* q = (uint4*)p;
+        int32_t t[52];
+#pragma unroll
+        for (int i = 0; i < 13; i++) t[i] = X.v[i], t[13 + i] = Y.v[i], t[26 + i] = Z.v[i], t[39 + i] = T.v[i];
+#pragma unroll
+        for (int i = 0; i < 13; i++) q[i] = make_uint4((uint32_t)t[4 * i], (uint32_t)t[4 * i + 1], (uint32_t)t[4 * i + 2], (uint32_t)t[4 * i + 3]);
+    }
+    SV_HD static void xyzz_from_raw(const g1_lazy_partial_t* p, fql_t& x, fql_t& y, fql_t& zz, fql_t& zzz) {
+        const uint4* q = (const uint4*)p;
+        int32_t t[52];
+#pragma unroll
+        for (int i = 0; i < 13; i++) {
+            const uint4 u = q[i];
+            t[4 * i] = (int32_t)u.x, t[4 * i + 1] = (int32_t)u.y, t[4 * i + 2] = (int32_t)u.z, t[4 * i + 3] = (int32_t)u.w;
+        }
+        fql_t X, Y, Z;
+#pragma unroll
+        for (int i = 0; i < 13; i++) X.v[i] = t[i], Y.v[i] = t[13 + i], Z.v[i] = t[26 + i];
+        const fql_t N = (Z + Y).normalized();
+        const fql_t D = Z - Y;
+        const fql_t z = fql_t::mul(D, X);
+        const fql_t cN = fql_t::mul(N, table(G1Ed::C));
+        const fql_t Xz = fql_t::mul(X, z);
+        x = fql_t::mul((cN - D).normalized(), Xz);
+        zz = fql_t::sqr(z);
+        zzz = fql_t::mul(zz, z);
+        const fql_t NZ = fql_t::mul(N, Z);
+        const fql_t cfNZ = fql_t::mul(NZ, table(G1Ed::CF));
+        y = fql_t::mul(cfNZ, zz);
+    }
+    SV_HD static g1_xyzz_t exact_xyzz_from_raw(const g1_lazy_partial_t* p) {
+        fql_t x, y, zz, zzz;
+        xyzz_from_raw(p, x, y, zz, zzz);
+        return {x.to_exact(), y.to_exact(), zz.to_exact(), zzz.to_exact()};
+    }
+};
+
+SV_HD bool g1_in_subgroup(const g1_aff_t& p) {
+    if (p.is_inf()) return true;
+    g1_xyzz_t acc = g1_xyzz_t::from_affine(p);
+#if defined(__HIP_DEVICE_COMPILE__)
+#pragma unroll 1
+#endif
+    for (int bit = 251; bit >= 0; bit--) {
+        acc = acc.dbl();
+        if ((G1Ed::ORDER[bit >> 5] >> (bit & 31)) & 1) acc.add_affine(p);
+    }
+    return acc.is_inf();
+}
+SV_HD fq_t g1_ed_const(const uint32_t* t) { return fq_t::from_table(t) * fq_t::from_table(FqLConv::C348); }
+struct g1_ed_fwd_t {
+    fq_t s, f, k2d, c406;
+    SV_HD static g1_ed_fwd_t make() { return {g1_ed_const(G1Ed::S), g1_ed_const(G1Ed::F), g1_ed_const(G1Ed::K2D), fq_t::from_table(FqLConv::C406)}; }
+    SV_HD fq_t den(const g1_aff_t& p) const {
+        if (p.is_inf()) return fq_t::one();
+        const fq_t u = s * (p.x + fq_t::one()), v = s * p.y;
+        return v * (u + fq_t::one());
+    }
+    SV_HD void slot(const g1_aff_t& p, const fq_t& inv_den, g1_ed_slot_t* out) const {
+        if (p.is_inf()) {
+            out->store(c406, c406, fq_t::zero());
+            return;
+        }
+        const fq_t u = s * (p.x + fq_t::one()), v = s * p.y;
+        const fq_t xe = f * u * (u + fq_t::one()) * inv_den;
+        const fq_t ye = (u - fq_t::one()) * v * inv_den;
+        out->store((ye - xe) * c406, (ye + xe) * c406, k2d * xe * ye * c406);
+    }
+};
+static constexpr int G1_ED_RUN = 8;
+SV_HD void g1_ed_convert_run(const g1_aff_mem_t* in, g1_ed_slot_t* out, int count) {
+    const g1_ed_fwd_t fw = g1_ed_fwd_t::make();
+    fq_t pre[G1_ED_RUN];
+    fq_t run = fq_t::one();
+    for (int i = 0; i < count; i++) {
+        pre[i] = run;
+        run = run * fw.den(g1_load_aff(&in[i]));
+    }
+    fq_t inv = run.inverse();
+    for (int i = count - 1; i >= 0; i--) {
+        const g1_aff_t p = g1_load_aff(&in[i]);
+        fw.slot(p, inv * pre[i], &out[i]);
+        inv = inv * fw.den(p);
+    }
+}
+
+}
diff --git a/snarkvm_amd/csrc/msm_sort.hip.h b/snarkvm_amd/csrc/msm_sort.hip.h
--- a/snarkvm_amd/csrc/msm_sort.hip.h
+++ b/snarkvm_amd/csrc/msm_sort.hip.h
@@ -2,6 +2,7 @@
 #include "ffl.hip.h"
 #include "ffl2.hip.h"
 #include "ffl2p.hip.h"
+#include "g1_edwards.hip.h"
 #include "msm.hip.h"
 
 namespace sv {
@@ -799,6 +800,79 @@
     }
 }
 
+template <bool PREFETCH>
+__global__ void __launch_bounds__(256, 1) msm_accumulate_ed_kernel(const g1_ed_slot_t* __restrict__ bases, const uint32_t* __restrict__ sorted,
+                                                            const uint32_t* __restrict__ boff, const uint32_t* __restrict__ start,
+                                                            g1_lazy_partial_t* __restrict__ partial, uint32_t nbt, uint32_t S, uint32_t debug_idx_mask) {
+    const uint32_t t = blockIdx.x * blockDim.x + threadIdx.x;
+    const uint32_t total = boff[nbt];
+    const uint64_t lo64 = (uint64_t)t * S;
+    if (lo64 >= total) return;
+    const uint32_t lo = (uint32_t)lo64;
+    const uint32_t hi = (total - lo < S) ? total : lo + S;
+    uint32_t k = find_bucket(boff, nbt, lo);
+    uint32_t kend = boff[k + 1];
+    uint32_t kend2 = boff[k + 2 <= nbt ? k + 2 : nbt];
+    uint32_t start_k = start[k];
+    uint32_t part_off = t - boff[k] / S;
+    ed_lazy_t acc = ed_lazy_t::identity();
+    auto slot_of = [&](uint32_t e) -> const g1_ed_slot_t* { return &bases[(e & 0x7fffffffu) & debug_idx_mask]; };
+    uint32_t e_cur = sorted[lo];
+    uint32_t e_n1 = lo + 1 < hi ? sorted[lo + 1] : 0u;
+    g1_ed_raw_t raw_next = g1_ed_raw_t::load(slot_of(e_cur));
+    for (uint32_t pos = lo;; pos++) {
+        const bool end = pos >= hi;
+        if (end || pos >= kend) {
+            acc.store_raw(&partial[start_k + part_off]);
+            if (end) break;
+            part_off = 0;
+            acc = ed_lazy_t::identity();
+            k++;
+            kend = kend2;
+            while (pos >= kend) {
+                k++;
+                kend = boff[k + 1];
+            }
+            kend2 = boff[k + 2 <= nbt ? k + 2 : nbt];
+            start_k = start[k];
+        }
+        const uint32_t e = e_cur;
+        const g1_ed_raw_t raw = raw_next;
+        if (pos + 1 < hi) raw_next = g1_ed_raw_t::load(slot_of(e_n1));
+        e_cur = e_n1;
+        if (pos + 2 < hi) e_n1 = sorted[pos + 2];
+        fql_t a0, a1, a2;
+        raw.operands(a0, a1, a2);
+        acc.madd(a0, a1, a2, (e >> 31) != 0);
+    }
+}
+template <bool LAZY>
+__global__ void __launch_bounds__(256) g1_ed_partials_convert_kernel(g1_lazy_partial_t* __restrict__ raw, g1_xyzz_mem_t* __restrict__ partial,
+                                                              const uint32_t* __restrict__ start, uint32_t nbt) {
+    const uint32_t i = blockIdx.x * blockDim.x + threadIdx.x;
+    if (i >= start[nbt]) return;
+    if constexpr (LAZY) {
+        xyzz_lazy_t r;
+        ed_lazy_t::xyzz_from_raw(&raw[i], r.x, r.y, r.zz, r.zzz);
+        r.inf = false;
+        r.store_raw(&raw[i]);
+    } else {
+        g1_store_xyzz(&partial[i], ed_lazy_t::exact_xyzz_from_raw(&raw[i]));
+    }
+}
+template <int V>
+__global__ void __launch_bounds__(256) g1_subgroup_check_kernel(const g1_aff_mem_t* __restrict__ slots, size_t n, uint32_t* __restrict__ bad) {
+    const size_t i = blockIdx.x * (size_t)blockDim.x + threadIdx.x;
+    if (i >= n) return;
+    if (!g1_in_subgroup(g1_load_aff(&slots[i]))) *bad = 1u;
+}
+template <int V>
+__global__ void __launch_bounds__(256) g1_bases_to_edwards_kernel(const g1_aff_mem_t* __restrict__ in, g1_ed_slot_t* __restrict__ out, size_t n) {
+    const size_t lo = (blockIdx.x * (size_t)blockDim.x + threadIdx.x) * G1_ED_RUN;
+    if (lo >= n) return;
+    g1_ed_convert_run(in + lo, out + lo, n - lo < (size_t)G1_ED_RUN ? (int)(n - lo) : G1_ED_RUN);
+}
+
 static __global__ void __launch_bounds__(256) g2_pair_partials_to_exact_kernel(const g2_pair_partial_t* __restrict__ raw, xyzz_mem_t<fq2_t>* __restrict__ partial,
                                                                         const uint32_t* __restrict__ start, uint32_t nbt) {
     const uint32_t g = blockIdx.x * blockDim.x + threadIdx.x;
diff --git a/snarkvm_amd/csrc/runtime.hip.h b/snarkvm_amd/csrc/runtime.hip.h
--- a/snarkvm_amd/csrc/runtime.hip.h
+++ b/snarkvm_amd/csrc/runtime.hip.h
@@ -378,6 +378,7 @@
     HIP_TRY(hipFuncSetAttribute((const void*)scan_one_block_kernel, hipFuncAttributeMaxDynamicSharedMemorySize, (int)(SCAN_ONE_MAX * 4)));
 #ifdef SV_TU_G1
     HIP_TRY(hipFuncSetAttribute((const void*)msm_accumulate_lazy_kernel<true>, hipFuncAttributeMaxDynamicSharedMemorySize, 128 * 1024));
+    HIP_TRY(hipFuncSetAttribute((const void*)msm_accumulate_ed_kernel<true>, hipFuncAttributeMaxDynamicSharedMemorySize, 128 * 1024));
 #endif
 #ifdef SV_TU_NTT
     HIP_TRY(hipFuncSetAttribute((const void*)ntt_pass_kernel_v2<false, ntt_arith_u>, hipFuncAttributeMaxDynamicSharedMemorySize, 96 * 1024));
@@ -635,6 +636,7 @@
     size_t n = 0;
     int tables = 1;
     int table_bits = 256;
+    int form = 0;
     mutable std::mutex co_mu;
     mutable std::condition_variable co_cv;
     mutable std::deque<msm_ticket_t*> co_q;
@@ -894,7 +896,7 @@
 }
 template <class F>
 static void msm_launch_accumulate(lane_t& c, const msm_plan_t& pl, const aff_mem_t<F>* vbase, uint32_t* boffp, uint32_t nbt, size_t nthreads, bool one_wave,
-                                  bool ltail) {
+                                  bool ltail, const g1_ed_slot_t* ed = nullptr) {
     hipStream_t st = c.stream;
 #ifdef SV_BENCH
     static const uint32_t dbg_mask = getenv("SNARKVM_HIP_DEBUG_IDX_MASK") ? (uint32_t)strtoul(getenv("SNARKVM_HIP_DEBUG_IDX_MASK"), nullptr, 0) : 0xffffffffu;
@@ -906,6 +908,17 @@
         if (msm_lazy_on<F>()) {
             if (!ltail) c.part_raw.ensure(tmax * sizeof(g1_lazy_partial_t));
             g1_lazy_partial_t* raw_out = ltail ? c.part_a.as<g1_lazy_partial_t>() : c.part_raw.as<g1_lazy_partial_t>();
+            if (ed) {
+                hipLaunchKernelGGL((msm_accumulate_ed_kernel<true>), dim3((unsigned)((nthreads + 255) / 256)), dim3(256), one_wave || tuning().acc_one_wg ? msm_acc_lds() : 0, st,
+                                   ed, c.sorted.as<uint32_t>(), boffp, c.start_a.as<uint32_t>(), raw_out, nbt, pl.S, dbg_mask);
+                if (ltail)
+                    hipLaunchKernelGGL((g1_ed_partials_convert_kernel<true>), dim3((unsigned)((tmax + 255) / 256)), dim3(256), 0, st, raw_out, (g1_xyzz_mem_t*)nullptr,
+                                       (const uint32_t*)c.start_a.as<uint32_t>(), nbt);
+                else
+                    hipLaunchKernelGGL((g1_ed_partials_convert_kernel<false>), dim3((unsigned)((tmax + 255) / 256)), dim3(256), 0, st, raw_out, c.part_a.as<g1_xyzz_mem_t>(),
+                                       (const uint32_t*)c.start_a.as<uint32_t>(), nbt);
+                return;
+            }
             hipLaunchKernelGGL((msm_accumulate_lazy_kernel<true>), dim3((unsigned)((nthreads + 255) / 256)), dim3(256), one_wave || tuning().acc_one_wg ? msm_acc_lds() : 0, st,
                                vbase, c.sorted.as<uint32_t>(), boffp, c.start_a.as<uint32_t>(), raw_out, nbt, pl.S, dbg_mask);
             if (!ltail)
@@ -941,6 +954,8 @@
 struct msm_job_t {
     const aff_mem_t<F>* bases = nullptr;
     const aff_mem_t<F>* bases1 = nullptr;
+    int form = 0;
+    const aff_mem_t<F>* form_origin = nullptr;
     size_t n0 = 0;
     int tables = 1;
     size_t table_stride = 0;
@@ -1231,7 +1246,9 @@
     if (mu && tuning().fuse_reduce < 0) rounds = mu->K >= 8 ? 1 : 0;
     hipLaunchKernelGGL(msm_alloc_seg_kernel, dim3((nbt + 1 + 255) / 256), dim3(256), 0, st, boffp, c.cnt_a.as<uint32_t>(), nbt, L.pl.S);
     exclusive_scan_u32(st, c.cnt_a.as<uint32_t>(), c.start_a.as<uint32_t>(), (size_t)nbt + 1, c.scan_tmp.as<uint32_t>());
-    msm_launch_accumulate<F>(c, L.pl, L.vbase, boffp, nbt, (L.E_max + L.pl.S - 1) / L.pl.S, L.single_round && L.prefetch_ok, L.ltail);
+    const g1_ed_slot_t* ed = nullptr;
+    if (sizeof(F) == sizeof(fq_t) && j.form == 1) ed = (const g1_ed_slot_t*)j.form_origin + (L.vbase - j.form_origin);
+    msm_launch_accumulate<F>(c, L.pl, L.vbase, boffp, nbt, (L.E_max + L.pl.S - 1) / L.pl.S, L.single_round && L.prefetch_ok, L.ltail, ed);
     ph.end();
     return rounds;
 }
@@ -1314,6 +1331,42 @@
     hipLaunchKernelGGL(g1_bases_to_form406_kernel, dim3((unsigned)((slots + 255) / 256)), dim3(256), 0, c.stream, d, slots);
     HIP_TRY(hipGetLastError());
 }
+template <int V = 0>
+static int g1_tables_to_msm_form(lane_t& c, g1_aff_mem_t** d, size_t n, int tables, double* check_ms = nullptr) {
+    const size_t slots = (size_t)tables * n;
+    if (!slots || !msm_lazy_on<fq_t>()) return 0;
+    if (tuning().edwards) {
+        const double t0 = host_now_ms();
+        c.scan_tmp.ensure(256);
+        uint32_t* d_bad = c.scan_tmp.as<uint32_t>();
+        uint32_t bad = 0;
+        HIP_TRY(hipMemsetAsync(d_bad, 0, 4, c.stream));
+        hipLaunchKernelGGL((g1_subgroup_check_kernel<V>), dim3((unsigned)((n + 255) / 256)), dim3(256), 0, c.stream, (const g1_aff_mem_t*)*d, n, d_bad);
+        HIP_TRY(hipGetLastError());
+        HIP_TRY(hipMemcpyAsync(&bad, d_bad, 4, hipMemcpyDeviceToHost, c.stream));
+        HIP_TRY(hipStreamSynchronize(c.stream));
+        if (check_ms) *check_ms = host_now_ms() - t0;
+        if (msm_trace_level() >= 1) fprintf(stderr, "[snarkvm_hip] register: subgroup test of %zu bases: %.2f ms, %s\n", n, host_now_ms() - t0, bad ? "failed" : "passed");
+        if (!bad) {
+            g1_ed_slot_t* ed = nullptr;
+            HIP_TRY(hipMalloc((void**)&ed, slots * sizeof(g1_ed_slot_t)));
+            const size_t threads = (slots + G1_ED_RUN - 1) / G1_ED_RUN;
+            hipLaunchKernelGGL((g1_bases_to_edwards_kernel<V>), dim3((unsigned)((threads + 255) / 256)), dim3(256), 0, c.stream, (const g1_aff_mem_t*)*d, ed, slots);
+            hipError_t e = hipGetLastError();
+            if (e == hipSuccess) e = hipStreamSynchronize(c.stream);
+            if (e != hipSuccess) {
+                (void)hipFree(ed);
+                HIP_TRY(e);
+            }
+            HIP_TRY(hipFree(*d));
+            *d = (g1_aff_mem_t*)ed;
+            return 1;
+        }
+    }
+    bases_to_lazy_form(c, *d, slots);
+    return 0;
+}
+static size_t g1_table_bytes(int form, size_t slots) { return slots * (form == 1 ? sizeof(g1_ed_slot_t) : sizeof(g1_aff_mem_t)); }
 #ifndef SV_NO_G2
 static void bases_to_lazy_form(lane_t& c, aff_mem_t<fq2_t>* d, size_t slots) {
     if (!slots || !msm_lazy_on<fq2_t>()) return;
@@ -1599,6 +1652,8 @@
     msm_job_t<F> j;
     j.bases = h.d[dev] + r.off0;
     j.bases1 = r.n1 ? h.d[dev] + r.off1 : nullptr;
+    j.form = h.form;
+    j.form_origin = h.d[dev];
     j.n0 = r.n0;
     j.tables = h.tables;
     j.table_stride = h.n;
diff --git a/snarkvm_amd/csrc/tuning.hip.h b/snarkvm_amd/csrc/tuning.hip.h
--- a/snarkvm_amd/csrc/tuning.hip.h
+++ b/snarkvm_amd/csrc/tuning.hip.h
@@ -6,7 +6,7 @@
 namespace sv {
 
 struct tuning_t {
-    int lazy = 1, lazy2 = 1, fused = 1;
+    int lazy = 1, lazy2 = 1, fused = 1, edwards = 1;
     long acc_lds = 96 * 1024;
     int acc_one_wg = 0, reduce_rounds = 1, fuse_batch = 1, fuse_max_k = 64, fuse_reduce = -1, coalesce = 1, coalesce_us = 40, lanes = 0;
     int msm_chunk_lg = 20, scalar_chunk_lg = 22, taper = 1, ring_lanes = 3, seg = 0, seg2 = 0, fold_l = 0, scan1 = 1;
@@ -19,7 +19,7 @@
         name = (decltype(name))v;          \
         return true;                       \
     }
-        SV_TUNE_KEY(lazy) SV_TUNE_KEY(lazy2) SV_TUNE_KEY(fused) SV_TUNE_KEY(acc_lds)
+        SV_TUNE_KEY(lazy) SV_TUNE_KEY(edwards) SV_TUNE_KEY(lazy2) SV_TUNE_KEY(fused) SV_TUNE_KEY(acc_lds)
         SV_TUNE_KEY(acc_one_wg) SV_TUNE_KEY(reduce_rounds) SV_TUNE_KEY(fuse_batch) SV_TUNE_KEY(fuse_max_k) SV_TUNE_KEY(fuse_reduce) SV_TUNE_KEY(coalesce)
         SV_TUNE_KEY(coalesce_us) SV_TUNE_KEY(lanes) SV_TUNE_KEY(msm_chunk_lg) SV_TUNE_KEY(scalar_chunk_lg) SV_TUNE_KEY(taper) SV_TUNE_KEY(ring_lanes) SV_TUNE_KEY(seg) SV_TUNE_KEY(seg2)
         SV_TUNE_KEY(fold_l) SV_TUNE_KEY(scan1) SV_TUNE_KEY(ntt_min_tiles) SV_TUNE_KEY(ntt_full_tw) SV_TUNE_KEY(ntt_fold)
diff --git a/snarkvm_amd/msm.py b/snarkvm_amd/msm.py
--- a/snarkvm_amd/msm.py
+++ b/snarkvm_amd/msm.py
@@ -82,6 +82,10 @@
         _lib.check(L.snarkvm_hip_msm_registered_batch(ctypes.c_void_p(out.ctypes.data), self._h, ctypes.c_size_t(count), c_offs, c_ns, c_ptrs,
                                                       ctypes.c_int(on_dev), ctypes.c_int(1 if montgomery else 0), ctypes.c_int(window_bits)))
         return out
+
+    @property
+    def bases_form(self):
+        return int(_lib.lib().snarkvm_hip_bases_form(self._h))
 
     def close(self):
         if self._h:
```
